# YuHang-max/3DSAD-main

Hardware: AMD Instinct MI355X
Metric: scenes/sec (16384-pt KITTI-shaped) through SA+cluster path (higher is better)
Workload: dtype f32

## Files before the change

### 3dsad-main_amd/_lib.py

```python
import ctypes
import os
import subprocess

_HERE = os.path.dirname(os.path.abspath(__file__))
CSRC = os.path.join(_HERE, "csrc")
SO_PATH = os.environ.get("SAD_AMD_LIB") or os.path.join(CSRC, "libsad_amd.so")

MAX_LAYERS = 4
MAX_RADII = 4
ABI_VERSION = 4
WS_REFILLS, WS_INUSE, WS_CONFLICT = 5, 6, 7

c_f32p = ctypes.POINTER(ctypes.c_float)
c_i32p = ctypes.POINTER(ctypes.c_int32)
vp = ctypes.c_void_p
c_i3p = ctypes.POINTER(ctypes.c_int)


class MlpArgs(ctypes.Structure):
    _fields_ = [
        ("struct_size", ctypes.c_size_t),
        ("xyz", vp), ("new_xyz", vp), ("idx", vp), ("cnt", vp), ("workspace", vp), ("feat", vp),
        ("ld_feat", ctypes.c_int),
        ("B", ctypes.c_int), ("N", ctypes.c_int), ("M", ctypes.c_int), ("S", ctypes.c_int),
# ... 57 lines not shown
        ("struct_size", ctypes.c_size_t),
        ("gt_boxes", vp), ("gt_labels", vp),
        ("B", ctypes.c_int), ("G", ctypes.c_int), ("D", ctypes.c_int), ("H", ctypes.c_int), ("W", ctypes.c_int),
        ("ns", ctypes.c_int), ("nr", ctypes.c_int), ("nb", ctypes.c_int), ("use_size_class", ctypes.c_int),
        ("sizes", ctypes.c_float * 48), ("z_center", ctypes.c_float * 16), ("rotations", ctypes.c_float * 8),
        ("pos_thr", ctypes.c_float * 16), ("neg_thr", ctypes.c_float * 16), ("size_class", ctypes.c_int32 * 16),
        ("x0", ctypes.c_float), ("y0", ctypes.c_float), ("sx", ctypes.c_float), ("sy", ctypes.c_float),
        ("dir_offset", ctypes.c_float),
        ("labels", vp), ("match", vp), ("reg_target", vp), ("max_iou", vp), ("dir_target", vp), ("workspace", vp),
    ]


class CenterTargetsArgs(ctypes.Structure):
    _fields_ = [
        ("struct_size", ctypes.c_size_t),
        ("gt_boxes", vp), ("gt_labels", vp),
        ("B", ctypes.c_int), ("G", ctypes.c_int), ("D", ctypes.c_int), ("C", ctypes.c_int), ("H", ctypes.c_int),
        ("W", ctypes.c_int), ("layout", ctypes.c_int), ("min_radius", ctypes.c_int), ("vel", ctypes.c_int),
        ("lo_x", ctypes.c_float), ("lo_y", ctypes.c_float), ("sx", ctypes.c_float), ("sy", ctypes.c_float),
        ("min_overlap", ctypes.c_float),
        ("heatmap", vp), ("ind", vp), ("anno", vp),
    ]


class AnchorHeadLossArgs(ctypes.Structure):
    _fields_ = [
        ("struct_size", ctypes.c_size_t),
        ("cls", vp), ("reg", vp), ("dir", vp), ("labels", vp), ("reg_target", vp), ("dir_target", vp),
        ("B", ctypes.c_int), ("H", ctypes.c_int), ("W", ctypes.c_int), ("A", ctypes.c_int), ("C", ctypes.c_int),
        ("nb", ctypes.c_int), ("layout", ctypes.c_int), ("sin_diff", ctypes.c_int), ("normalize", ctypes.c_int),
        ("alpha", ctypes.c_float), ("beta", ctypes.c_float),
        ("code_weights", ctypes.c_float * 7), ("scale", ctypes.c_float * 3),
        ("loss", vp), ("num_pos", vp), ("grad_cls", vp), ("grad_reg", vp), ("grad_dir", vp), ("per_anchor", vp),
        ("workspace", vp),
    ]


class CenterHeadLossArgs(ctypes.Structure):
    _fields_ = [
        ("struct_size", ctypes.c_size_t),
        ("hm", vp), ("reg", vp), ("height", vp), ("dim", vp), ("rot", vp), ("vel", vp),
        ("heatmap", vp), ("ind", vp), ("anno", vp),
        ("B", ctypes.c_int), ("H", ctypes.c_int), ("W", ctypes.c_int), ("C", ctypes.c_int), ("G", ctypes.c_int),
        ("layout", ctypes.c_int), ("normalize", ctypes.c_int),
        ("code_weights", ctypes.c_float * 10), ("scale", ctypes.c_float * 2),
        ("loss", vp), ("num_pos", vp),
        ("grad_hm", vp), ("grad_reg", vp), ("grad_height", vp), ("grad_dim", vp), ("grad_rot", vp), ("grad_vel", vp),
        ("workspace", vp),
    ]


ROI_CLS_MODES = {"roi_iou": 0, "cls": 1}


class RoiTargetsArgs(ctypes.Structure):
    _fields_ = [
        ("struct_size", ctypes.c_size_t),
        ("rois", vp), ("roi_count", vp), ("roi_labels", vp), ("gt_boxes", vp), ("gt_labels", vp),
        ("B", ctypes.c_int), ("R", ctypes.c_int), ("D", ctypes.c_int), ("G", ctypes.c_int), ("Dg", ctypes.c_int),
        ("S", ctypes.c_int), ("fg_max", ctypes.c_int), ("cls_mode", ctypes.c_int), ("seed", ctypes.c_uint),
        ("fg_thr", ctypes.c_float), ("bg_lo", ctypes.c_float), ("hard_ratio", ctypes.c_float), ("reg_fg_thr", ctypes.c_float),
        ("cls_fg_thr", ctypes.c_float), ("cls_bg_thr", ctypes.c_float),
        ("index", vp), ("match", vp), ("labels", vp), ("iou", vp), ("cls_target", vp), ("reg_valid", vp),
        ("rois_s", vp), ("gt_local", vp), ("reg_target", vp), ("workspace", vp),
    ]


class RoiHeadLossArgs(ctypes.Structure):
    _fields_ = [
        ("struct_size", ctypes.c_size_t),
        ("rcnn_cls", vp), ("rcnn_reg", vp), ("cls_target", vp), ("reg_valid", vp), ("reg_target", vp), ("rois", vp), ("gt_local", vp),
        ("B", ctypes.c_int), ("S", ctypes.c_int), ("D", ctypes.c_int), ("normalize", ctypes.c_int),
        ("beta", ctypes.c_float), ("code_weights", ctypes.c_float * 7), ("scale", ctypes.c_float * 3),
        ("loss", vp), ("num", vp), ("grad_cls", vp), ("grad_reg", vp), ("grad_corner", vp), ("per_roi", vp),
    ]


SIGNATURES = {
    "sad_version": (ctypes.c_int, []),
    "sad_last_error": (ctypes.c_char_p, []),
    "sad_set_option": (ctypes.c_int, [ctypes.c_char_p, ctypes.c_int]),
    "sad_fps_workspace_bytes": (ctypes.c_size_t, [ctypes.c_int, ctypes.c_int]),
    "sad_fps_f32": (ctypes.c_int, [vp, ctypes.c_int, ctypes.c_int, ctypes.c_int, vp, vp, vp]),
    "sad_ffps_workspace_bytes": (ctypes.c_size_t, [ctypes.c_int, ctypes.c_int]),
    "sad_pairdist_f32": (ctypes.c_int, [vp, vp, ctypes.c_int, ctypes.c_int, ctypes.c_int, ctypes.c_int,
                                       ctypes.c_float, vp, vp]),
    "sad_ffps_f32": (ctypes.c_int, [vp, vp] + [ctypes.c_int] * 5 + [ctypes.c_float, vp, vp, vp]),
    "sad_gather_xyz_f32": (ctypes.c_int, [vp, vp, ctypes.c_int, ctypes.c_int, ctypes.c_int, vp, vp]),
    "sad_gather_points": (ctypes.c_int, [vp, vp] + [ctypes.c_int] * 5 + [vp, vp]),
    "sad_group_points": (ctypes.c_int, [vp, vp] + [ctypes.c_int] * 6 + [vp, vp]),
    "sad_group_points_grad_f32": (ctypes.c_int, [vp, vp] + [ctypes.c_int] * 5 + [vp, vp]),
    "sad_group_points_grad_pm_f32": (ctypes.c_int, [vp, vp] + [ctypes.c_int] * 5 + [vp, vp]),
    "sad_max_pool_s_f32": (ctypes.c_int, [vp] + [ctypes.c_int] * 4 + [vp, vp, vp]),
    "sad_max_pool_s_grad_f32": (ctypes.c_int, [vp, vp] + [ctypes.c_int] * 4 + [vp, vp]),
    "sad_ball_query_f32": (ctypes.c_int, [vp, vp, ctypes.c_float, vp] + [ctypes.c_int] * 4 + [vp, vp]),
    "sad_ball_query_multi_f32": (ctypes.c_int, [vp, vp, ctypes.c_int, c_f32p, vp,
                                               ctypes.POINTER(ctypes.c_int), ctypes.POINTER(vp),
                                               ctypes.POINTER(vp),
                                               ctypes.c_int, ctypes.c_int, ctypes.c_int, vp]),
    "sad_ball_query_grid_workspace_bytes": (ctypes.c_size_t, [ctypes.c_int, ctypes.c_int]),
    "sad_ball_query_grid_f32": (ctypes.c_int, [vp, vp, ctypes.c_int, c_f32p, ctypes.POINTER(ctypes.c_int),
                                              ctypes.POINTER(vp), ctypes.POINTER(vp),
                                              ctypes.c_int, ctypes.c_int, ctypes.c_int, vp, vp]),
    "sad_subsample_pad_f32": (ctypes.c_int, [vp, vp, ctypes.c_int, ctypes.c_int, ctypes.c_int, ctypes.c_uint, vp, vp]),
    "sad_copy_rows_u32": (ctypes.c_int, [vp, ctypes.c_longlong, vp, ctypes.c_longlong, ctypes.c_longlong, ctypes.c_longlong, vp]),
    "sad_knn_f32": (ctypes.c_int, [vp, vp] + [ctypes.c_int] * 4 + [vp, vp]),
    "sad_three_nn_f32": (ctypes.c_int, [vp, vp] + [ctypes.c_int] * 3 + [vp, vp, vp, vp]),
    "sad_three_interpolate_f32": (ctypes.c_int, [vp, vp, vp] + [ctypes.c_int] * 5 + [vp, ctypes.c_int, ctypes.c_int, vp]),
    "sad_three_interpolate_grad_f32": (ctypes.c_int, [vp, vp, vp] + [ctypes.c_int] * 5 + [vp, vp]),
    "sad_boxes_iou_f32": (ctypes.c_int, [vp, vp] + [ctypes.c_int] * 6 + [vp, vp]),
    "sad_points_in_boxes_f32": (ctypes.c_int, [vp, vp] + [ctypes.c_int] * 4 + [vp, vp]),
    "sad_roipoint_pool3d_f32": (ctypes.c_int, [vp, vp, vp] + [ctypes.c_int] * 5 + [ctypes.c_float, ctypes.c_int, vp, vp, vp, vp]),
    "sad_voxel_workspace_bytes": (ctypes.c_int, [ctypes.c_int] * 3 + [ctypes.POINTER(ctypes.c_size_t)]),
    "sad_voxel_coords_f32": (ctypes.c_int, [vp, vp] + [ctypes.c_int] * 3 + [c_f32p, c_f32p, vp, vp]),
    "sad_voxel_index_f32": (ctypes.c_int, [vp, vp] + [ctypes.c_int] * 3 + [c_f32p, c_f32p, ctypes.c_int, vp, vp, vp, vp, vp, vp]),
    "sad_voxelize_f32": (ctypes.c_int, [vp, vp] + [ctypes.c_int] * 3 + [c_f32p, c_f32p, ctypes.c_int, ctypes.c_int, vp, vp, vp, vp, vp, vp]),
    "sad_voxel_reduce_f32": (ctypes.c_int, [vp, vp, vp] + [ctypes.c_int] * 5 + [vp, vp, vp, vp, vp]),
    "sad_voxel_reduce_grad_f32": (ctypes.c_int, [vp, vp, vp] + [ctypes.c_int] * 5 + [vp, vp, vp]),
    "sad_voxel_encode_workspace_bytes": (ctypes.c_int, [ctypes.c_int] * 5 + [ctypes.POINTER(ctypes.c_size_t)]),
    "sad_voxel_decorate_f32": (ctypes.c_int, [vp] * 5 + [ctypes.c_int] * 5 + [c_f32p, c_f32p, ctypes.c_int, ctypes.c_int, vp, vp, vp]),
    "sad_voxel_encode_f32": (ctypes.c_int, [vp] * 5 + [ctypes.c_int] * 5 + [c_f32p, c_f32p, vp, vp] + [ctypes.c_int] * 3 + [vp] * 5),
    "sad_spconv_workspace_bytes": (ctypes.c_int, [ctypes.c_int, ctypes.c_int, c_i3p, c_i3p, ctypes.c_int, ctypes.POINTER(ctypes.c_size_t)]),
    "sad_spconv_index_subm": (ctypes.c_int, [vp, vp, ctypes.c_int, ctypes.c_int, c_i3p, c_i3p, vp, vp, vp]),
    "sad_spconv_index_count": (ctypes.c_int, [vp, vp, ctypes.c_int, ctypes.c_int, c_i3p, c_i3p, c_i3p, c_i3p, vp, vp, vp]),
    "sad_spconv_index_fill": (ctypes.c_int, [vp, vp, ctypes.c_int, ctypes.c_int, c_i3p, c_i3p, c_i3p, c_i3p, vp, ctypes.c_int, vp, vp, vp, vp]),
    "sad_spconv_packed_floats": (ctypes.c_size_t, [ctypes.c_int] * 3),
    "sad_spconv_pack_f32": (ctypes.c_int, [vp, vp] + [ctypes.c_int] * 3 + [vp, vp]),
    "sad_spconv_f32": (ctypes.c_int, [vp, vp, vp, vp] + [ctypes.c_int] * 6 + [vp, vp]),
    "sad_sparse_to_dense_workspace_bytes": (ctypes.c_int, [ctypes.c_int, c_i3p, ctypes.POINTER(ctypes.c_size_t)]),
    "sad_sparse_to_dense_f32": (ctypes.c_int, [vp, vp, vp] + [ctypes.c_int] * 3 + [c_i3p, vp, vp, vp]),
    "sad_spconv_index_transpose": (ctypes.c_int, [vp] + [ctypes.c_int] * 3 + [vp, vp, vp]),
    "sad_spconv_grad_weight_workspace_bytes": (ctypes.c_int, [ctypes.c_int] * 4 + [ctypes.POINTER(ctypes.c_size_t)]),
    "sad_spconv_grad_weight_f32": (ctypes.c_int, [vp, vp, vp] + [ctypes.c_int] * 5 + [vp, vp, vp, vp]),
    "sad_spconv_max_pool_f32": (ctypes.c_int, [vp, vp] + [ctypes.c_int] * 4 + [vp, vp, vp]),
    "sad_spconv_max_pool_grad_f32": (ctypes.c_int, [vp, vp, vp] + [ctypes.c_int] * 4 + [vp, vp]),
    "sad_mlp_packed_floats": (ctypes.c_size_t, [ctypes.c_int, ctypes.POINTER(ctypes.c_int), ctypes.c_int]),
    "sad_mlp_pack_f32": (ctypes.c_int, [ctypes.c_int, ctypes.POINTER(ctypes.c_int), ctypes.c_int,
                                       ctypes.POINTER(vp), ctypes.POINTER(vp), vp, vp]),
    "sad_mlp_workspace_bytes": (ctypes.c_size_t, [ctypes.c_int, ctypes.c_int, ctypes.c_int]),
    "sad_mlp_rowscan": (ctypes.c_int, [ctypes.c_int, ctypes.POINTER(vp), ctypes.POINTER(vp), ctypes.POINTER(ctypes.c_int),
                                       ctypes.c_int, ctypes.c_int, ctypes.c_int, ctypes.POINTER(vp), vp]),
    "sad_mlp_rowscan_init": (ctypes.c_int, [ctypes.c_int, ctypes.POINTER(vp), ctypes.POINTER(vp), ctypes.POINTER(ctypes.c_int),
                                            ctypes.c_int, ctypes.c_int, ctypes.c_int, ctypes.POINTER(vp), ctypes.POINTER(vp),
                                            ctypes.POINTER(ctypes.c_int), ctypes.POINTER(ctypes.c_int), ctypes.POINTER(ctypes.c_int), vp]),
    "sad_mlp_rowscan_split": (ctypes.c_int, [ctypes.c_int, ctypes.POINTER(vp), ctypes.POINTER(vp), ctypes.POINTER(ctypes.c_int),
                                             ctypes.c_int, ctypes.c_int, ctypes.c_int, ctypes.POINTER(vp), ctypes.POINTER(vp),
                                             ctypes.POINTER(ctypes.c_int), vp]),
    "sad_mlp_cont_bytes": (ctypes.c_size_t, [ctypes.c_int] * 4),
    "sad_mlp_preferred_geometry": (ctypes.c_int, [ctypes.c_int, ctypes.POINTER(ctypes.c_int)]),
    "sad_mlp_padded_dims": (ctypes.c_int, [ctypes.c_int, ctypes.POINTER(ctypes.c_int), ctypes.POINTER(ctypes.c_int)]),
    "sad_mlp_scratch_bytes": (ctypes.c_size_t, [ctypes.c_int, ctypes.c_int, ctypes.c_int, ctypes.c_int,
                                               ctypes.POINTER(ctypes.c_int)]),
    "sad_mlp_chain_f32": (ctypes.c_int, [ctypes.POINTER(MlpArgs), vp]),
    "sad_mlp_chain_multi_f32": (ctypes.c_int, [ctypes.POINTER(ctypes.POINTER(MlpArgs)), ctypes.c_int, vp]),
    "sad_mlp_packed_bytes_bf16": (ctypes.c_size_t, [ctypes.c_int, ctypes.POINTER(ctypes.c_int), ctypes.c_int]),
    "sad_mlp_pack_bf16": (ctypes.c_int, [ctypes.c_int, ctypes.POINTER(ctypes.c_int), ctypes.c_int,
                                        ctypes.POINTER(vp), ctypes.POINTER(vp), vp, vp]),
    "sad_mlp_preferred_geometry_bf16": (ctypes.c_int, [ctypes.c_int, ctypes.POINTER(ctypes.c_int)]),
    "sad_mlp_chain_bf16": (ctypes.c_int, [ctypes.POINTER(MlpBf16Args), vp]),
    "sad_mlp_chain_multi_bf16": (ctypes.c_int, [ctypes.POINTER(ctypes.POINTER(MlpBf16Args)), ctypes.c_int, vp]),
    "sad_candidates_f32": (ctypes.c_int, [vp, vp, ctypes.c_int, ctypes.c_int, ctypes.c_int,
                                         ctypes.c_float, ctypes.c_float, ctypes.c_float, c_f32p,
                                         vp, vp, vp]),
    "sad_nms_bev_f32": (ctypes.c_int, [vp, ctypes.c_int, ctypes.c_int, ctypes.c_float, ctypes.c_float,
                                      vp, vp, vp, vp]),
    "sad_nms_bev_workspace_bytes": (ctypes.c_size_t, [ctypes.c_int, ctypes.c_int]),
    "sad_nms_bev_ws_f32": (ctypes.c_int, [vp, ctypes.c_int, ctypes.c_int, ctypes.c_float, ctypes.c_float,
                                         vp, vp, vp, vp, vp]),
    "sad_nms_boxes_workspace_bytes": (ctypes.c_size_t, [ctypes.c_int] * 3),
    "sad_nms_boxes_f32": (ctypes.c_int, [vp, ctypes.c_int, vp, vp, ctypes.c_int, ctypes.c_int, ctypes.c_float, ctypes.c_float,
                                        ctypes.c_int, ctypes.c_int, vp, vp, vp, vp, vp]),
    "sad_decode_boxes_f32": (ctypes.c_int, [vp, vp, ctypes.c_int, ctypes.c_int, c_f32p, vp, vp]),
    "sad_anchor_decode_f32": (ctypes.c_int, [ctypes.POINTER(AnchorDecodeArgs), vp]),
    "sad_center_decode_f32": (ctypes.c_int, [ctypes.POINTER(CenterDecodeArgs), vp]),
    "sad_anchor_targets_workspace_bytes": (ctypes.c_size_t, [ctypes.c_int, ctypes.c_int]),
    "sad_anchor_targets_f32": (ctypes.c_int, [ctypes.POINTER(AnchorTargetsArgs), vp]),
    "sad_center_targets_f32": (ctypes.c_int, [ctypes.POINTER(CenterTargetsArgs), vp]),
    "sad_anchor_head_loss_workspace_bytes": (ctypes.c_size_t, [ctypes.c_int] * 4),
    "sad_anchor_head_loss_f32": (ctypes.c_int, [ctypes.POINTER(AnchorHeadLossArgs), vp]),
    "sad_center_head_loss_workspace_bytes": (ctypes.c_size_t, [ctypes.c_int] * 4),
    "sad_center_head_loss_f32": (ctypes.c_int, [ctypes.POINTER(CenterHeadLossArgs), vp]),
    "sad_roi_targets_workspace_bytes": (ctypes.c_size_t, [ctypes.c_int, ctypes.c_int]),
    "sad_roi_targets_f32": (ctypes.c_int, [ctypes.POINTER(RoiTargetsArgs), vp]),
    "sad_roi_decode_f32": (ctypes.c_int, [vp, ctypes.c_int, vp, ctypes.c_int, ctypes.c_int, vp, vp]),
    "sad_roi_head_loss_f32": (ctypes.c_int, [ctypes.POINTER(RoiHeadLossArgs), vp]),
}

_lib = None

import threading
_tls = threading.local()


def recorder():
    return getattr(_tls, "rec", None)


def set_recorder(rec) -> None:
    _tls.rec = rec


def is_launch(name: str) -> bool:
    return (name.startswith("sad_") and not name.endswith(("_bytes", "_floats", "_bytes_bf16"))
            and "preferred_geometry" not in name and name not in ("sad_version", "sad_last_error", "sad_set_option", "sad_mlp_padded_dims"))


def build(force: bool = False) -> str:
    cmd = ["make", "-C", CSRC, "-j4"] + (["-B"] if force else [])
    subprocess.check_call(cmd, stdout=subprocess.DEVNULL)
    return SO_PATH


def lib():
    global _lib
    if _lib is None:
        if not os.path.exists(SO_PATH):
            raise RuntimeError(
                f"{SO_PATH} is missing: build it with `python -c 'import __graft_entry__ as g; "
                "g.build()'` (hipcc, gfx950).  sad_amd has no CPU fallback.")
        import torch
        handle = ctypes.CDLL(SO_PATH)
        for name, (res, args) in SIGNATURES.items():
            fn = getattr(handle, name)
            fn.restype = res
            fn.argtypes = args
        if handle.sad_version() != ABI_VERSION:
            raise RuntimeError(f"{SO_PATH}: ABI version {handle.sad_version()}, this binding needs {ABI_VERSION} "
                               "(stale build: run __graft_entry__.build())")
        _lib = handle
    rec = getattr(_tls, "rec", None)
    return _lib if rec is None else rec.lib


def check(code: int, what: str) -> None:
    if code != 0:
        msg = lib().sad_last_error()
        raise RuntimeError(f"{what} failed ({code}): {msg.decode() if msg else ''}")


def set_option(key: str, value: int) -> None:
    check(lib().sad_set_option(key.encode(), int(value)), "sad_set_option")
```

### 3dsad-main_amd/csrc/api.hip

```cpp
#include <string.h>

#include "common.h"

namespace sad {

static thread_local char g_err[512] = "";
static std::atomic<int> g_opt[OPT_COUNT] = {};

void set_error(const char *fmt, ...) {
    va_list ap;
    va_start(ap, fmt);
    vsnprintf(g_err, sizeof g_err, fmt, ap);
    va_end(ap);
}

int get_option(int which) { return (which >= 0 && which < OPT_COUNT) ? g_opt[which].load(std::memory_order_relaxed) : 0; }

}

SAD_API int sad_version(void) { return SAD_ABI_VERSION; }

SAD_API const char *sad_last_error(void) { return sad::g_err; }

SAD_API int sad_set_option(const char *key, int value) {
    SAD_REQUIRE(key, "sad_set_option: NULL key");
    if (!strcmp(key, "fps_dpp")) { sad::g_opt[sad::OPT_FPS_DPP].store(value, std::memory_order_relaxed); return SAD_OK; }
    if (!strcmp(key, "mlp_rw")) { sad::g_opt[sad::OPT_MLP_RW].store(value, std::memory_order_relaxed); return SAD_OK; }
    if (!strcmp(key, "mlp_budget_kb")) { sad::g_opt[sad::OPT_MLP_BUDGET_KB].store(value, std::memory_order_relaxed); return SAD_OK; }
    if (!strcmp(key, "mlp_force")) { sad::g_opt[sad::OPT_MLP_FORCE].store(value, std::memory_order_relaxed); return SAD_OK; }
    if (!strcmp(key, "mlp_dedup_f")) { sad::g_opt[sad::OPT_MLP_DEDUP_F].store(value, std::memory_order_relaxed); return SAD_OK; }
    if (!strcmp(key, "mlp_nodedup")) { sad::g_opt[sad::OPT_MLP_NODEDUP].store(value, std::memory_order_relaxed); return SAD_OK; }
    if (!strcmp(key, "mlp_static")) { sad::g_opt[sad::OPT_MLP_STATIC].store(value, std::memory_order_relaxed); return SAD_OK; }
    if (!strcmp(key, "mlp_noxcd")) { sad::g_opt[sad::OPT_MLP_NOXCD].store(value, std::memory_order_relaxed); return SAD_OK; }
    if (!strcmp(key, "mlp_dyn_slots")) { sad::g_opt[sad::OPT_MLP_DYN_SLOTS].store(value, std::memory_order_relaxed); return SAD_OK; }
    if (!strcmp(key, "mlp_steal_after")) { sad::g_opt[sad::OPT_MLP_STEAL_AFTER].store(value, std::memory_order_relaxed); return SAD_OK; }
    if (!strcmp(key, "mlp_layer_queue")) { sad::g_opt[sad::OPT_MLP_LAYER_QUEUE].store(value, std::memory_order_relaxed); return SAD_OK; }
    if (!strcmp(key, "mlp_rows_form")) { sad::g_opt[sad::OPT_MLP_ROWS_FORM].store(value, std::memory_order_relaxed); return SAD_OK; }
    if (!strcmp(key, "mlp_check_inuse")) { sad::g_opt[sad::OPT_MLP_CHECK_INUSE].store(value, std::memory_order_relaxed); return SAD_OK; }
    if (!strcmp(key, "group_variant")) { sad::g_opt[sad::OPT_GROUP_VARIANT].store(value, std::memory_order_relaxed); return SAD_OK; }
    if (!strcmp(key, "bq_variant")) { sad::g_opt[sad::OPT_BQ_VARIANT].store(value, std::memory_order_relaxed); return SAD_OK; }
    if (!strcmp(key, "fps_threads")) { sad::g_opt[sad::OPT_FPS_THREADS].store(value, std::memory_order_relaxed); return SAD_OK; }
    if (!strcmp(key, "nn_variant")) { sad::g_opt[sad::OPT_NN_VARIANT].store(value, std::memory_order_relaxed); return SAD_OK; }
    if (!strcmp(key, "spconv_grad_ranges")) { sad::g_opt[sad::OPT_SPCONV_GRAD_RANGES].store(value, std::memory_order_relaxed); return SAD_OK; }
    if (!strcmp(key, "fps_variant")) { sad::g_opt[sad::OPT_FPS_VARIANT].store(value, std::memory_order_relaxed); return SAD_OK; }
    return sad::fail(SAD_EINVAL, "sad_set_option: unknown key '%s'", key);
}
```

### 3dsad-main_amd/csrc/common.h

```cpp
#pragma once
#include <hip/hip_runtime.h>
#include <atomic>
#include <stdarg.h>
#include <stdint.h>
#include <stdio.h>

#include "../../include/sad_amd.h"

#define SAD_API extern "C" __attribute__((visibility("default")))

namespace sad {

void set_error(const char *fmt, ...);
int get_option(int which);
struct ScanJob {
    const int32_t *cnt, *idx;
    int *tab, *blk_sum, *row_src, *row_gid;
    int ngroups, S, N, M, nodedup, R, blk0;
    float *zout;
    int zld, zcols;
    int split;
    int *gstart;
    void *cont0;
    int cont_cols;
};
struct ScanLayout { long long blk_sum, row_src, row_gid, gstart, ints; };
inline ScanLayout scan_layout(long long ng, int S) {
    ScanLayout t;
    t.blk_sum = 4 + (ng + 1);
    t.row_src = t.blk_sum + (ng * S / 32 + 2) + (ng / 1024 + 2);
    t.row_gid = t.row_src + ng * S;
    t.gstart = (t.row_gid + ng * S + 3) & ~3LL;
    t.ints = t.gstart + ng + 1;
    return t;
}
inline void scan_zero_fill(ScanJob &jb, float *out, int ld_out, int col_off, int cols) { jb.zout = out + col_off; jb.zld = ld_out; jb.zcols = cols; }
inline void heaviest_first(const double *weight, int n, int *order) {
    for (int i = 0; i < n; ++i) order[i] = i;
    for (int i = 0; i < n; ++i)
        for (int k = i + 1; k < n; ++k)
            if (weight[order[k]] > weight[order[i]]) { const int t = order[i]; order[i] = order[k]; order[k] = t; }
}
constexpr int CONT_BIT = 1 << 29;
constexpr int GID_MASK = CONT_BIT - 1;
constexpr int SCAN_MAX_CHAINS = SAD_MAX_RADII;
struct ScanMulti { ScanJob j[SCAN_MAX_CHAINS]; int n; };
ScanJob make_scan_job(const int32_t *cnt, int ngroups, int S, int R, int *tab, int nodedup, const int32_t *idx, int N, int M);
int launch_rowscan_multi(const ScanJob *jobs, int n, hipStream_t st);
int launch_rowscan(const int32_t *cnt, int ngroups, int S, int R, int *tab, hipStream_t st, int nodedup = 0,
                   const int32_t *idx = nullptr, int N = 0, int M = 1);
int launch_fps_cellg(const float *xyz, int B, int N, int M, int32_t *idx, void *workspace, hipStream_t st);
int launch_fps_bucket(const float *xyz, int B, int N, int M, int32_t *idx, void *workspace, hipStream_t st);
constexpr int REG_MAX_CHAINS = 3;
struct RegChain {
    const float *xyz, *new_xyz, *feat, *packed;
    float *out;
    const int *rowtab;
    const int *row_src, *row_gid;
    long long off[3];
    long long stream_off;
    int np[3];
    int ld_feat, C, cpr;
    int ld_out, col_off, cout_last, vec_out;
};
struct RegMulti {
    RegChain c[REG_MAX_CHAINS];
    int shape[REG_MAX_CHAINS];
    int n;
    int *counter;
    int nq;
    long long max_tiles;
    int steal_after;
    int check_id;
};
struct LayerJob {
    const float *x;
    const float *xyz, *new_xyz;
    const int *rowtab, *row_src, *row_gid;
    int rows;
    const float *packed;
    long long off;
    int ldx, np, kg, nog;
    int cpr, gather, relu, last;
    float *y;
    int ldy;
    float *out;
    int ld_out, col_off, cout_last;
};
struct LayerMulti {
    LayerJob j[2];
    int n;
    int *queue;
};
int launch_layers(const LayerMulti &lm, long long max_items, hipStream_t st);
int *stream_item_queue(hipStream_t st);
struct RowsJob {
    const float *x;
    int ldx;
    long long rows;
    const float *packed;
    long long off;
    int np, kg, ct, cout;
    int relu;
    float *out;
    int ld_out, col_off, vec_out;
    int nrb, ncb;
};
int launch_rows(const RowsJob &job, hipStream_t st);
int reg_shape_id(int L, const int *kp, const int *np);
int reg_family(int shape);
int launch_reg(const RegMulti &mp, hipStream_t st);
bool coop_shape(int shape);
long long coop_stream_frags(int shape, const int *kp, const int *np);
int launch_coop(const RegMulti &mp, hipStream_t st);
struct BfRegChain {
    const float *xyz, *new_xyz;
    const void *feat;
    int feat_bf16, ld_feat, C;
    const void *stream;
    int stream_frags;
    const float *bias[3];
    int np[3];
    float *out;
    int ld_out, col_off, cout_last;
    const int *rowtab, *row_src, *row_gid;
    int out_bf16, ld_cont;
    void *cont;
};
struct BfRegMulti {
    BfRegChain c[REG_MAX_CHAINS];
    int shape[REG_MAX_CHAINS];
    int n;
    long long max_tiles;
    int static_f4;
};
struct BfRowsJob {
    const void *x;
    int x_bf16, ldx, kin;
    long long rows;
    const void *w;
    const float *bias;
    int ks, ct, cout;
    int relu;
    void *out;
    int out_bf16, ld_out, col_off, vec_out;
    int nrb, ncb;
    int n_pool;
    const int *pool_gstart[SAD_MAX_RADII];
    const void *pool_cont[SAD_MAX_RADII];
    int pool_col0[SAD_MAX_RADII + 1];
    int pool_ld[SAD_MAX_RADII];
};
int launch_bf16_rows(const BfRowsJob &job, hipStream_t st);
int bfreg_shape_id(int L, const int *dims);
int bfreg_family(int shape);
long long bfreg_stream_frags(int shape);
int bfreg_pack(int shape, const int *dims, int first_has_xyz, const float *const *W, void *dst, hipStream_t st);
int launch_bfreg(const BfRegMulti &mp, hipStream_t st);
enum { OPT_FPS_DPP = 0, OPT_MLP_RW = 1, OPT_MLP_BUDGET_KB = 2, OPT_BQ_VARIANT = 3, OPT_FPS_VARIANT = 4, OPT_MLP_FORCE = 5, OPT_MLP_DEDUP_F = 6, OPT_MLP_NODEDUP = 7, OPT_FPS_THREADS = 8, OPT_MLP_STATIC = 9, OPT_GROUP_VARIANT = 10, OPT_MLP_DYN_SLOTS = 11, OPT_MLP_NOXCD = 12, OPT_MLP_STEAL_AFTER = 13, OPT_MLP_CHECK_INUSE = 14, OPT_MLP_LAYER_QUEUE = 15, OPT_MLP_ROWS_FORM = 16, OPT_NN_VARIANT = 17, OPT_SPCONV_GRAD_RANGES = 18, OPT_COUNT };

inline int fail(int code, const char *fmt, ...) {
    char buf[480];
    va_list ap;
    va_start(ap, fmt);
    vsnprintf(buf, sizeof buf, fmt, ap);
    va_end(ap);
    set_error("%s", buf);
    return code;
}

inline int device_cus() {
    static std::atomic<int> cached{0};
    int c = cached.load(std::memory_order_relaxed);
    if (c > 0) return c;
    int dev = 0;
    c = 256;
    if (hipGetDevice(&dev) == hipSuccess) {
        int v = 0;
        if (hipDeviceGetAttribute(&v, hipDeviceAttributeMultiprocessorCount, dev) == hipSuccess && v > 0) c = v;
    }
    (void)hipGetLastError();
    cached.store(c, std::memory_order_relaxed);
    return c;
}

inline void lds_attr_once(std::atomic<uint64_t> &done, const void *fn, int bytes) {
    int dev = 0;
    if (hipGetDevice(&dev) != hipSuccess) { (void)hipGetLastError(); return; }
    const uint64_t bit = 1ull << (dev & 63);
    if (done.load(std::memory_order_acquire) & bit) return;
    if (hipFuncSetAttribute(fn, hipFuncAttributeMaxDynamicSharedMemorySize, bytes) != hipSuccess) (void)hipGetLastError();
    done.fetch_or(bit, std::memory_order_release);
}

__host__ __device__ inline size_t al16(size_t x) { return (x + 15) & ~(size_t)15; }
struct Carve {
    size_t o = 0;
    size_t take(size_t bytes) { const size_t at = o; o += al16(bytes); return at; }
};
inline unsigned blocks_for(unsigned long long n, int threads) { return (unsigned)((n + threads - 1) / threads); }

inline int check_launch(const char *what) {
    hipError_t e = hipGetLastError();
    if (e != hipSuccess) return fail(SAD_ELAUNCH, "%s: %s", what, hipGetErrorString(e));
    return SAD_OK;
}

constexpr int ITEMQ_REFILLS = 3, ITEMQ_INUSE = 4, ITEMQ_CONFLICT = 5;
struct ItemQueue {
    int *q;
    int nq, own;
};
constexpr int ITEMQ_INTS = 2 + 32 * 8;
__device__ __forceinline__ ItemQueue itemq_init(int *q, int nq) {
    unsigned xcc = 0;
    if (nq == 8) asm volatile("s_getreg_b32 %0, hwreg(HW_REG_XCC_ID)" : "=s"(xcc));
    return ItemQueue{q, nq, (int)(xcc & 7u)};
}
__device__ __forceinline__ int *itemq_counter(const ItemQueue &Q, int x) { return Q.nq == 8 ? Q.q + 2 + 32 * x : Q.q; }
__device__ __forceinline__ int itemq_item(const ItemQueue &Q, int x, int pos) { return Q.nq == 8 ? pos * 8 + x : pos; }
__device__ __forceinline__ int itemq_pull(const ItemQueue &Q, int n = 1) { return atomicAdd(itemq_counter(Q, Q.own), n); }
__device__ __forceinline__ int itemq_steal(const ItemQueue &Q, int nitems) {
    if (Q.nq != 8) return nitems;
    int seen[7];
#pragma unroll
    for (int k = 0; k < 7; ++k)
        seen[k] = __hip_atomic_load(itemq_counter(Q, (Q.own + 1 + k) & 7), __ATOMIC_RELAXED, __HIP_MEMORY_SCOPE_AGENT);
#pragma unroll
    for (int k = 0; k < 7; ++k) {
        const int x = (Q.own + 1 + k) & 7;
        if (itemq_item(Q, x, seen[k]) >= nitems) continue;
        const int it = itemq_item(Q, x, atomicAdd(itemq_counter(Q, x), 1));
        if (it < nitems) return it;
    }
    return nitems;
}
__device__ __forceinline__ void itemq_done(const ItemQueue &Q, int workgroups) {
    if (atomicAdd(Q.q + 1, 1) != workgroups - 1) return;
    Q.q[0] = 0;
    Q.q[1] = 0;
    if (Q.nq == 8) {
        for (int x = 0; x < 8; ++x) Q.q[2 + 32 * x] = 0;
        Q.q[ITEMQ_INUSE] = 0;
    }
}
__device__ __forceinline__ void itemq_claim(const ItemQueue &Q, int id) {
    if (Q.nq != 8 || id == 0) return;
    const int old = atomicCAS(Q.q + ITEMQ_INUSE, 0, id);
    if (old != 0 && old != id) atomicExch(Q.q + ITEMQ_CONFLICT, 1);
}

__device__ __forceinline__ float d2f(float px, float py, float pz, float cx, float cy, float cz) {
    float dx = px - cx, dy = py - cy, dz = pz - cz;
    float xx = dx * dx, yy = dy * dy, zz = dz * dz;
    float s = xx + yy;
    return s + zz;
}

}

#define SAD_REQUIRE(cond, ...)                                \
    do {                                                      \
        if (!(cond)) return sad::fail(SAD_EINVAL, __VA_ARGS__); \
    } while (0)

template <class T> int args_ok(const char *fn, const T *a) {
    SAD_REQUIRE(a, "%s: NULL args", fn);
    SAD_REQUIRE(a->struct_size == sizeof(T), "%s: struct_size %zu, this library has %zu", fn, a->struct_size, sizeof(T));
    return SAD_OK;
}
```

### 3dsad-main_amd/csrc/mlp_chain.h

```cpp
#pragma once
#include "common.h"

namespace sad {
namespace chain {

constexpr int MAXL = SAD_MAX_LAYERS;
constexpr int WHOLE_BIT = 1 << 30;

struct MlpParams {
    const float *xyz;
    const float *new_xyz;
    const int32_t *idx;
    const int32_t *cnt;
    const float *feat;
    const float *packed;
    float *out;
    long long total_rows;
    int ld_feat, N, M, S, C;
    int sp_shift;
    int grouped;
    int L;
    int kp[MAXL];
    int np[MAXL];
    int cout_last;
    long long off[MAXL];
    int relu_mask;
    int ld_out, col_off;
    int wn_shift;
    int xcd_nb;
    int flex;
    int kc;
    int bufA_rows, bufB_rows;
    int cpr, cshift;
    int vec_out;
    int bias_total;
    int G;
    int nodedup;
    int s_off_entries;
    int *rowtab;
    const int *row_src, *row_gid;
    long long total_groups;
};

constexpr int MULTI_MAX = 4;
struct MultiParams {
    MlpParams p[MULTI_MAX];
    int first[MULTI_MAX + 1];
    int rw[MULTI_MAX];
    int cw[MULTI_MAX];
    int n;
};

struct ValuParams {
    const float *xyz, *new_xyz, *feat;
    const int32_t *idx, *cnt;
    const float *w[3], *b[3];
    float *out;
    long long total_groups;
    int ld_feat, N, M, S, G, nodedup, ld_out, col_off, vec_out;
};
constexpr int VALU_T = 256;
constexpr int VALU_GMAX = 2048;

struct Geometry {
    int kp[MAXL], np[MAXL];
    long long off[MAXL];
    long long raw_w[MAXL];
    long long raw_b[MAXL];
    long long stream_off;
    long long stream_frags;
    long long total;
};
Geometry geometry(int L, const int *dims, int first_has_xyz);
int check_dims(const char *fn, int L, const int *dims);

int launch_tiled(const MlpParams &p, int W, int RW, int CW, size_t lds, long long nblocks, hipStream_t st);
int launch_tiled_multi(const MultiParams &mp, int W, int rwmax, bool cw2, size_t lds, hipStream_t st);
int launch_valu(const ValuParams &v, int shape, long long nblocks, hipStream_t st);

}
}
```

### 3dsad-main_amd/csrc/mlp_chain.hip

```cpp
#include "common.h"
#include "mlp_chain.h"

namespace {

using namespace sad::chain;

#include "prims.h"

#ifndef SAD_MLP_BDEPTH
#define SAD_MLP_BDEPTH 2
#endif

__device__ __forceinline__ int act_idx(int c, int r, int PS) {
    return (((c >> 3) << 1) + (c & 1)) * PS + r * 4 + ((c & 7) >> 1);
}

template <int CTRL>
__device__ __forceinline__ float dpp_max(float v) {
    const float o = __builtin_bit_cast(float, __builtin_amdgcn_update_dpp(0, __builtin_bit_cast(int, v), CTRL, 0xF, 0xF, false));
    return o > v ? o : v;
}

__device__ __forceinline__ float group_max(float v, int steps) {
    if (steps > 0) v = dpp_max<0xB1>(v);
// ... 110 lines not shown
                a0[u] = lda(af0, t + D + u, n4);
                a1[u] = lda(af1, t + D + u, n4);
                const int tb = t + u + 2;
                b[u % 2] = bp[(tb < n4 ? tb : n4 - 1) * kbs];
                __builtin_amdgcn_sched_barrier(0);
            }
        }
    }
    const int rem = n4 - t;
#pragma unroll
    for (int u = 0; u < D - 1; ++u) {
        if (u < rem) {
            mma4x2(acc0, acc1, a0[u], a1[u], b[u % 2]);
            if (u + 2 < rem) b[u % 2] = bp[(t + u + 2) * kbs];
        }
    }
}
__device__ __forceinline__ int s_off_last_group(const int *s_off, int G, int T) {
    int lo = 0, hi = G;
    while (hi - lo > 1) {
        const int mid = (lo + hi) >> 1;
        if (s_off[mid] <= T - 1) lo = mid; else hi = mid;
    }
    return lo;
}

template <int W, int RW, int CW = 1>
__device__ __forceinline__ void mlp_chain_body(const MlpParams &p, const int block_in) {
    static_assert(CW == 1 || RW == 1, "two output tiles per wave only with one row tile");
    int block = block_in;
    if (p.xcd_nb > 0) {
        const int per = (p.xcd_nb + 7) >> 3;
        block = (block_in & 7) * per + (block_in >> 3);
        if (block >= p.xcd_nb) return;
    }
    extern __shared__ __attribute__((aligned(16))) float smem[];
    const int tid = threadIdx.x;
    const int lane = tid & 63;
    const int j = lane & 31, h = lane >> 5;
    const int wave = __builtin_amdgcn_readfirstlane(tid >> 6);
    const int WN = 1 << p.wn_shift;
    const int WM = W >> p.wn_shift;
    const int wn = wave & (WN - 1);
    const int wm = wave >> p.wn_shift;
    const int R = 32 * RW * WM;
    const int PS = 4 * R + 8;
    float *bufA = smem;
    float *bufB = smem + (size_t)(p.bufA_rows >> 2) * PS;
    float *sbias = bufB + (size_t)(p.bufB_rows >> 2) * PS;
    int *sm_idx = reinterpret_cast<int *>(sbias + p.bias_total);
    int *sm_gid = sm_idx + R;
    int *s_off = sm_gid + R;
    const int koff = p.grouped ? 4 : 0;

    {
        int bo = 0;
        for (int l = 0; l < p.L; ++l) {
            for (int c = tid; c < p.np[l]; c += W * 64) sbias[bo + c] = p.packed[p.off[l] + c];
            bo += p.np[l];
        }
    }
    long long r0 = (long long)block * R;
    long long g0 = 0;
    int T = R, npass = 1, G = p.G;
    const bool dyn = p.grouped && p.rowtab != nullptr;
    int &s_pass = s_off[p.s_off_entries];
    if (p.grouped && !dyn) {
        g0 = (long long)block * p.G;
        long long left = p.total_groups - g0;
        const int ng = (int)(left < p.G ? left : p.G);
        if (p.cnt) {
            for (int gi = tid; gi < p.G; gi += W * 64) {
                int cnt = 0;
                if (gi < ng) {
                    cnt = p.cnt[g0 + gi];
                    cnt = cnt < 1 ? 1 : (cnt > p.S ? p.S : cnt);
                    if (p.nodedup) cnt = p.S;
                }
                s_off[gi + 1] = cnt;
            }
        } else {
            for (int gi = wave; gi < p.G; gi += W) {
                int cnt = 0;
                if (gi < ng) {
                    const int32_t *ip = p.idx + (g0 + gi) * p.S;
                    const int v = lane < p.S ? ip[lane] : 0;
                    const int first = __builtin_amdgcn_readfirstlane(v);
                    const unsigned long long diff = __ballot(lane < p.S && v != first);
                    cnt = diff ? 64 - __builtin_clzll(diff) : 1;
                    if (p.nodedup) cnt = p.S;
                }
                if (lane == 0) s_off[gi + 1] = cnt;
            }
        }
        if (tid == 0) s_off[0] = 0;
        __syncthreads();
        if (wave == 0) {
            int carry = 0;
            for (int base = 0; base < p.G; base += 64) {
                const int gi = base + lane;
                int v = gi < p.G ? s_off[gi + 1] : 0;
                for (int off = 1; off < 64; off <<= 1) {
                    const int u = __shfl_up(v, off, 64);
                    if (lane >= off) v += u;
                }
                if (gi < p.G) s_off[gi + 1] = v + carry;
                carry += __builtin_amdgcn_readlane(v, 63);
            }
        }
        __syncthreads();
        T = s_off[p.G];
        npass = (T + R - 1) / R;
    }
    const int nchunks = (p.kp[0] + p.kc - 1) / p.kc;

    int next_pass = 0;
    if (dyn && tid == 0) s_pass = atomicAdd(p.rowtab + 2, 1);
    for (int pass_i = 0; dyn || pass_i < npass; ++pass_i) {
        int pass = pass_i;
        int qoff = pass * R;
        if (dyn) {
            __syncthreads();
            pass = s_pass;
            const int total = p.rowtab[0];
            if (pass >= p.rowtab[1]) break;
            T = total - pass * R < R ? total - pass * R : R;
            qoff = 0;
            g0 = 0;
            for (int r = tid; r < R; r += W * 64) {
                const bool valid = r < T;
                const int q = pass * R + (valid ? r : T - 1);
                sm_idx[r] = p.row_src[q];
                const int gv = p.row_gid[q];
                sm_gid[r] = valid ? gv : ~gv;
            }
        }
        for (int r = tid; r < R && !dyn; r += W * 64) {
            if (p.grouped) {
                int q = qoff + r;
                const bool valid = dyn ? r < T : q < T;
                if (!valid) q = T - 1;
                int lo = 0, hi = G;
                while (hi - lo > 1) {
                    const int mid = (lo + hi) >> 1;
                    if (s_off[mid] <= q) lo = mid; else hi = mid;
                }
                const long long gg = g0 + lo;
                const int b = (int)(gg / p.M);
                sm_idx[r] = (int)((long long)b * p.N + p.idx[gg * p.S + (q - s_off[lo])]);
                sm_gid[r] = valid ? lo : -1;
            } else {
                long long gr = r0 + r;
                if (gr >= p.total_rows) gr = p.total_rows - 1;
                sm_idx[r] = (int)gr;
            }
        }
        __syncthreads();
        if (dyn && tid == 0) next_pass = atomicAdd(p.rowtab + 2, 1);

        int bias_off = 0;
        for (int l = 0; l < p.L; ++l) {
            const float *in = (l & 1) ? bufB : bufA;
            float *outb = (l & 1) ? bufA : bufB;
            const int n_oc = p.np[l] >> 5;
            const int nrounds = p.flex ? (n_oc * WM + W * CW - 1) / (W * CW) : (n_oc + WN * CW - 1) / (WN * CW);
            const float4 *frags = reinterpret_cast<const float4 *>(p.packed + p.off[l] + p.np[l]);
            const int nT4 = p.kp[l] >> 3;
            const bool last = (l == p.L - 1);
            const bool relu = (p.relu_mask >> l) & 1;
            const int lchunks = (l == 0) ? nchunks : 1;
            const int keep = last ? p.cout_last : p.kp[l + 1];

            for (int round = 0; round < nrounds; ++round) {
                int ocs[CW];
                bool haves[CW];
                int rtb = wm * RW;
#pragma unroll
                for (int c = 0; c < CW; ++c) {
                    const int item = wave + (round * CW + c) * W;
                    ocs[c] = p.flex ? item / WM : wn + ((round * CW + c) << p.wn_shift);
                    if (p.flex) rtb = item - ocs[c] * WM;
                    haves[c] = ocs[c] < n_oc;
                }
                const bool have = haves[0];
                f32x16 accs[CW][RW];
#pragma unroll
                for (int c = 0; c < CW; ++c) {
                    if (!haves[c]) continue;
#pragma unroll
                    for (int a = 0; a < 4; ++a) {
                        const float4 bv = *reinterpret_cast<const float4 *>(sbias + bias_off + ocs[c] * 32 + 8 * a + 4 * h);
#pragma unroll
                        for (int rt = 0; rt < RW; ++rt) {
                            accs[c][rt][4 * a + 0] = bv.x;
                            accs[c][rt][4 * a + 1] = bv.y;
                            accs[c][rt][4 * a + 2] = bv.z;
                            accs[c][rt][4 * a + 3] = bv.w;
                        }
                    }
                }
                for (int ck = 0; ck < lchunks; ++ck) {
                    const int k0 = (l == 0) ? ck * p.kc : 0;
                    int k1 = (l == 0) ? k0 + p.kc : p.kp[l];
                    if (k1 > p.kp[l]) k1 = p.kp[l];
                    if (l == 0 && (round == 0 || lchunks > 1)) {
                        if (!(round == 0 && ck == 0)) __syncthreads();
                        if (p.grouped && k0 == 0) {
                            for (int r = tid; r < R; r += W * 64) {
                                const int gv = sm_gid[r];
                                const int gi = dyn ? ((gv < 0 ? ~gv : gv) & (WHOLE_BIT - 1))
                                                   : (gv < 0 ? s_off_last_group(s_off, G, T) : gv);
                                const float *q = p.xyz + (long long)sm_idx[r] * 3;
                                const float *c = p.new_xyz + (g0 + gi) * 3;
                                *reinterpret_cast<float2 *>(bufA + r * 4) = make_float2(q[0] - c[0], q[2] - c[2]);
                                *reinterpret_cast<float2 *>(bufA + PS + r * 4) = make_float2(q[1] - c[1], 0.f);
                            }
                        }
                        const int f0 = (k0 > koff ? k0 : koff) - koff;
                        const int f1 = k1 - koff;
                        const int fl = f1 < p.C ? f1 : p.C;
                        if (p.cpr > 0) {
                            const int cprp = 1 << p.cshift;
                            const int rpp = 64 >> p.cshift;
                            for (int r = wave * rpp + (lane >> p.cshift); r < R; r += W * rpp) {
                                const float *src = p.feat + (long long)sm_idx[r] * p.ld_feat;
                                for (int ch = (f0 >> 2) + (lane & (cprp - 1)); ch < (fl >> 2); ch += cprp) {
                                    const float4 v = *reinterpret_cast<const float4 *>(src + 4 * ch);
                                    const int c = koff + 4 * ch - k0;
                                    float *d = bufA + (size_t)((c >> 3) << 1) * PS + r * 4 + ((c & 7) >> 1);
                                    *reinterpret_cast<float2 *>(d) = make_float2(v.x, v.z);
                                    *reinterpret_cast<float2 *>(d + PS) = make_float2(v.y, v.w);
                                }
                            }
                        } else {
                            for (int r = tid; r < R; r += W * 64) {
                                const float *src = p.feat + (long long)sm_idx[r] * p.ld_feat;
                                for (int c = f0; c < fl; ++c) bufA[act_idx(koff + c - k0, r, PS)] = src[c];
                            }
                        }
                        const int z0 = (koff + p.C > k0 ? koff + p.C : k0);
                        for (int k = z0 + wave; k < k1; k += W)
                            for (int r = lane; r < R; r += 64) bufA[act_idx(k - k0, r, PS)] = 0.f;
                        __syncthreads();
                    }
                    if (have) {
                        const float4 *bp = reinterpret_cast<const float4 *>(in) + (size_t)h * (PS >> 2) + rtb * 32 + j;
                        const float4 *af = frags + ((size_t)ocs[0] * nT4 + (k0 >> 3)) * 64 + lane;
                        if constexpr (CW == 2) {
                            if (haves[CW - 1]) {
                                const float4 *af1 = frags + ((size_t)ocs[CW - 1] * nT4 + (k0 >> 3)) * 64 + lane;
                                mma_ktile2<SAD_MLP_ADEPTH>(accs[0][0], accs[CW - 1][0], af, af1, (k1 - k0) >> 3, bp, PS >> 1);
                            } else {
                                mma_ktile<RW, SAD_MLP_ADEPTH>(accs[0], af, (k1 - k0) >> 3, bp, PS >> 1);
                            }
                        } else {
                            mma_ktile<RW, SAD_MLP_ADEPTH>(accs[0], af, (k1 - k0) >> 3, bp, PS >> 1);
                        }
                    }
                }
#pragma unroll
                for (int cw = 0; cw < CW; ++cw) {
                if (!haves[cw]) continue;
                const int oc = ocs[cw];
                f32x16 (&acc)[RW] = accs[cw];
                if (relu) {
#pragma unroll
                    for (int rt = 0; rt < RW; ++rt)
#pragma unroll
                        for (int g = 0; g < 16; ++g) acc[rt][g] = acc[rt][g] > 0.f ? acc[rt][g] : 0.f;
                }
                if (!last) {
#pragma unroll
                    for (int a = 0; a < 4; ++a) {
                        if (oc * 32 + 8 * a >= keep) continue;
#pragma unroll
                        for (int rt = 0; rt < RW; ++rt) {
                            float *d = outb + (size_t)((oc * 4 + a) * 2) * PS + ((rtb + rt) * 32 + j) * 4 + 2 * h;
                            *reinterpret_cast<float2 *>(d) = make_float2(acc[rt][4 * a + 0], acc[rt][4 * a + 2]);
                            *reinterpret_cast<float2 *>(d + PS) = make_float2(acc[rt][4 * a + 1], acc[rt][4 * a + 3]);
                        }
                    }
                } else if (!p.grouped) {
#pragma unroll
                    for (int rt = 0; rt < RW; ++rt) {
                        const long long gr = r0 + (rtb + rt) * 32 + j;
                        if (gr >= p.total_rows) continue;
                        float *o = p.out + gr * p.ld_out + p.col_off;
#pragma unroll
                        for (int a = 0; a < 4; ++a) {
                            const int ch = oc * 32 + 8 * a + 4 * h;
                            if (p.vec_out && ch + 3 < p.cout_last) {
                                *reinterpret_cast<float4 *>(o + ch) = make_float4(acc[rt][4 * a], acc[rt][4 * a + 1], acc[rt][4 * a + 2], acc[rt][4 * a + 3]);
                            } else {
#pragma unroll
                                for (int e = 0; e < 4; ++e)
                                    if (ch + e < p.cout_last) o[ch + e] = acc[rt][4 * a + e];
                            }
                        }
                    }
                } else {
#pragma unroll
                    for (int rt = 0; rt < RW; ++rt) {
                        const int rbase = (rtb + rt) * 32;
                        const int gid = sm_gid[rbase + j];
                        int same[5];
#pragma unroll
                        for (int st = 0; st < 5; ++st) {
// ... 268 lines not shown
```

### 3dsad-main_amd/csrc/mlp_dispatch.hip

```cpp
#include "mlp_chain.h"

using namespace sad::chain;

namespace {
enum Kind { VALU_DONE, TILED, REG, COOP, ROWS, LAYERED };
struct Prepared {
    Kind kind;
    MlpParams p;
    size_t lds;
    long long nblocks;
    int W, RW, CW;
    sad::RegChain rc;
    int reg_shape;
    long long reg_tiles;
    sad::ScanJob scan;
    bool prescanned;
    sad::RowsJob rj;
    sad::LayerJob lj[MAXL];
    int nl;
    long long layer_items[MAXL];
};
struct Chain {
    const sad_mlp_args *a;
    Geometry g;
// ... 228 lines not shown
        return ((size_t)((ra + rb) / 4) * (4 * R + 8) + 2 * R + nso + (size_t)bias_total) * 4 + 16;
    };
    const int bkb = sad::get_option(sad::OPT_MLP_BUDGET_KB);
    const size_t BUDGET2 = (size_t)(bkb > 0 ? bkb : 78) * 1024, BUDGET1 = 156 * 1024;
    int W = 8, wn_shift = 0, RW = 1, kc = g.kp[0];
    if (const int geom = c.geom_wg) {
        const int fw = geom / 100, fwns = (geom / 10) % 10, frw = geom % 10;
        const bool ok = (fw == 4 || fw == 8 || fw == 16) && (1 << fwns) <= fw && (frw == 1 || frw == 2 || frw == 4);
        if (!ok) return sad::fail(SAD_EUNSUPPORTED, "sad_mlp_chain_f32: geometry %d is not valid here", geom);
        W = fw; wn_shift = fwns; RW = frw;
        if (lds_bytes(W, wn_shift, RW, kc) > BUDGET1) {
            kc = g.kp[0] < 256 ? g.kp[0] : 256;
            if (kc == g.kp[0] || lds_bytes(W, wn_shift, RW, kc) > BUDGET1)
                return sad::fail(SAD_EUNSUPPORTED, "sad_mlp_chain_f32: geometry %d does not fit LDS", geom);
        }
    } else {
        double wsum = 0, fsum = 0;
        for (int l = 0; l < a->L; ++l) {
            const double f = (double)g.kp[l] * g.np[l];
            wsum += f * (g.np[l] / 32);
            fsum += f;
        }
        int wns0 = 0;
        while (wns0 < 3 && (2 << wns0) <= wsum / fsum + 1e-9) ++wns0;
        bool found = false;
        for (int pass = 0; pass < 3 && !found; ++pass) {
            const size_t budget = pass == 0 ? BUDGET2 : BUDGET1;
            const int kcc = pass < 2 ? g.kp[0] : (g.kp[0] < 256 ? g.kp[0] : 256);
            for (int wns = wns0; wns <= 3 && !found; ++wns) {
                int best_rw = 0;
                for (int rw = 4; rw >= 1; rw >>= 1) {
                    if (lds_bytes(8, wns, rw, kcc) > budget) continue;
                    if (!best_rw) best_rw = rw;
                    const long long R = 32LL * rw * (8 >> wns);
                    const long long nb = grouped ? (p.total_groups * a->S / dedup_f + R - 1) / R : (p.total_rows + R - 1) / R;
                    if (nb >= 1024 || rw == 1) { best_rw = rw; break; }
                }
                if (best_rw) { wn_shift = wns; RW = best_rw; kc = kcc; found = true; }
            }
        }
        if (!found) return sad::fail(SAD_EUNSUPPORTED, "sad_mlp_chain_f32: layer widths do not fit LDS");
    }
    p.wn_shift = wn_shift;
    if (flex_code > 3 || (flex_code && RW != 1))
        return sad::fail(SAD_EUNSUPPORTED, "sad_mlp_chain_f32: flexible distribution / two tiles per wave need RW == 1");
    if ((flex_code & 2) && W == 16) return sad::fail(SAD_EUNSUPPORTED, "sad_mlp_chain_f32: two tiles per wave: 4 or 8 waves");
    p.flex = flex_code & 1;
    p.kc = kc;
    lds_rows(kc, p.bufA_rows, p.bufB_rows);
    const size_t lds = lds_bytes(W, wn_shift, RW, kc);
    const long long R = 32LL * RW * (W >> wn_shift);
    p.G = grouped ? groups_per_wg((int)R) : 0;
    p.s_off_entries = (int)((p.G > R + 1 ? p.G : R + 1) + 1);
    p.nodedup = sad::get_option(sad::OPT_MLP_NODEDUP);
    p.rowtab = nullptr;
    long long grid_dyn = 0;
    long long macs_per_row = 0;
    for (int l = 0; l < a->L; ++l) macs_per_row += (long long)g.kp[l] * g.np[l];
    const bool want_dyn = c.dyn_code == 1 || (c.dyn_code == 0 && p.total_groups <= 16384 && macs_per_row >= 400000);
    if (grouped && a->cnt && a->workspace && want_dyn && !sad::get_option(sad::OPT_MLP_STATIC)) {
        SAD_REQUIRE((uintptr_t)a->workspace % 16 == 0, "sad_mlp_chain_f32: workspace must be 16-byte aligned");
        SAD_REQUIRE(p.total_groups < (1LL << 30), "sad_mlp_chain_f32: too many groups");
        p.rowtab = (int *)a->workspace;
        if (int e = sad::launch_rowscan(a->cnt, (int)p.total_groups, a->S, (int)R, p.rowtab, (hipStream_t)stream, p.nodedup,
                                        a->idx, a->N, a->M)) return e;
        const sad::ScanLayout t = sad::scan_layout(p.total_groups, a->S);
        p.row_src = p.rowtab + t.row_src;
        p.row_gid = p.rowtab + t.row_gid;
        const long long upper = (p.total_groups * a->S + R - 1) / R;
        long long per_cu = lds > 80 * 1024 ? 1 : (lds > 52 * 1024 ? 2 : (lds > 39 * 1024 ? 3 : 4));
        if (sad::get_option(sad::OPT_MLP_DYN_SLOTS) > 0 && sad::get_option(sad::OPT_MLP_DYN_SLOTS) < per_cu)
            per_cu = sad::get_option(sad::OPT_MLP_DYN_SLOTS);
        grid_dyn = upper < 256 * per_cu ? upper : 256 * per_cu;
    }
    const long long nblocks = grid_dyn ? grid_dyn : (grouped ? (p.total_groups + p.G - 1) / p.G : (p.total_rows + R - 1) / R);
    SAD_REQUIRE(nblocks < (1LL << 31), "sad_mlp_chain_f32: too many workgroups");
    if (W == 16 && RW == 4) return sad::fail(SAD_EUNSUPPORTED, "sad_mlp_chain_f32: 16 waves support RW 1 or 2");
    q.kind = TILED;
    q.p = p; q.lds = lds; q.nblocks = nblocks; q.W = W; q.RW = RW; q.CW = (flex_code & 2) ? 2 : 1;
    if (!grid_dyn && !sad::get_option(sad::OPT_MLP_NOXCD)) {
        q.p.xcd_nb = (int)nblocks;
        q.nblocks = ((nblocks + 7) / 8) * 8;
    }
    return SAD_OK;
}

static int prepare_chain(const sad_mlp_args *a, sad_stream_t stream, Prepared &q) {
    Chain c;
    if (int e = chain_args(a, c)) return e;
    q.prescanned = a->prescanned != 0;
    switch (c.geom_wg) {
    case 1: return prepare_valu(c, stream, q);
    case 2: case 4: return prepare_reg(c, q);
    case 3: return prepare_layered(c, q);
    case 5: return prepare_rows(c, q);
    default: return prepare_tiled(c, stream, q);
    }
}

namespace {
int launch_pending_scans(const Prepared *const *qs, int n, hipStream_t st) {
    sad::ScanJob jobs[sad::REG_MAX_CHAINS];
    int m = 0;
    for (int i = 0; i < n; ++i)
        if (!qs[i]->prescanned) jobs[m++] = qs[i]->scan;
    return m ? sad::launch_rowscan_multi(jobs, m, st) : SAD_OK;
}

int launch_reg_chains(const Prepared *const *qs, int n, hipStream_t st) {
    sad::RegMulti mp{};
    mp.n = n;
    mp.max_tiles = 0;
    if (int e = launch_pending_scans(qs, n, st)) return e;
    for (int i = 0; i < n; ++i) {
        mp.c[i] = qs[i]->rc;
        mp.shape[i] = qs[i]->reg_shape;
        mp.max_tiles += qs[i]->reg_tiles;
    }
    mp.counter = const_cast<int *>(mp.c[0].rowtab) + 2;
    mp.nq = qs[0]->scan.ngroups + 1 >= sad::ITEMQ_INTS ? 8 : 1;
    return qs[0]->kind == COOP ? sad::launch_coop(mp, st) : sad::launch_reg(mp, st);
}

int launch_layered_chains(const Prepared *const *qs, int n, hipStream_t st) {
    if (int e = launch_pending_scans(qs, n, st)) return e;
    for (int l = 0; l < qs[0]->nl; ++l) {
        sad::LayerMulti lm{};
        lm.n = n;
        long long items = 0;
        for (int i = 0; i < n; ++i) { lm.j[i] = qs[i]->lj[l]; items += qs[i]->layer_items[l]; }
        if (int e = sad::launch_layers(lm, items, st)) return e;
    }
    return SAD_OK;
}

int launch_prepared(const Prepared &q, hipStream_t st) {
    const Prepared *one = &q;
    switch (q.kind) {
    case VALU_DONE: return SAD_OK;
    case ROWS: return sad::launch_rows(q.rj, st);
    case LAYERED: return launch_layered_chains(&one, 1, st);
    case REG: case COOP: return launch_reg_chains(&one, 1, st);
    default: return launch_tiled(q.p, q.W, q.RW, q.CW, q.lds, q.nblocks, st);
    }
}
}

SAD_API int sad_mlp_chain_f32(const sad_mlp_args *a, sad_stream_t stream) {
    Prepared q;
    if (int e = prepare_chain(a, stream, q)) return e;
    return launch_prepared(q, (hipStream_t)stream);
}

SAD_API int sad_mlp_chain_multi_f32(const sad_mlp_args *const *args, int n, sad_stream_t stream) {
    SAD_REQUIRE(args && n >= 1, "sad_mlp_chain_multi_f32: need at least one chain");
    hipStream_t st = (hipStream_t)stream;
    if (n > MULTI_MAX) {
        for (int i = 0; i < n; i += MULTI_MAX)
            if (int e = sad_mlp_chain_multi_f32(args + i, n - i < MULTI_MAX ? n - i : MULTI_MAX, stream)) return e;
        return SAD_OK;
    }
    Prepared q[MULTI_MAX];
    for (int i = 0; i < n; ++i)
        if (int e = prepare_chain(args[i], stream, q[i])) return e;
    if (n == 2 && q[0].kind == LAYERED && q[1].kind == LAYERED && q[0].nl == q[1].nl) {
        const int last = q[0].nl - 1;
        const bool swap = q[1].layer_items[last] * (long long)q[1].lj[last].kg > q[0].layer_items[last] * (long long)q[0].lj[last].kg;
        const Prepared *ord[2] = {swap ? &q[1] : &q[0], swap ? &q[0] : &q[1]};
        return launch_layered_chains(ord, 2, st);
    }
    double weight[MULTI_MAX];
    int order[MULTI_MAX];
    bool all_reg = n > 1 && n <= sad::REG_MAX_CHAINS && (q[0].kind == REG || q[0].kind == COOP);
    for (int i = 0; i < n; ++i) all_reg = all_reg && q[i].kind == q[0].kind && sad::reg_family(q[i].reg_shape) == sad::reg_family(q[0].reg_shape);
    if (all_reg) {
        for (int i = 0; i < n; ++i) {
            double m = 0;
            for (int l = 0; l < 3; ++l) m += (double)q[i].rc.np[l] * (l == 0 ? 8.0 * 17 : q[i].rc.np[l - 1]);
            weight[i] = m * (double)q[i].reg_tiles;
        }
        sad::heaviest_first(weight, n, order);
        const Prepared *ord[MULTI_MAX];
        for (int i = 0; i < n; ++i) ord[i] = &q[order[i]];
        return launch_reg_chains(ord, n, st);
    }
    bool merge = n > 1;
    for (int i = 0; i < n; ++i) merge = merge && q[i].kind == TILED && q[i].W == q[0].W && q[i].W != 16;
    if (!merge) {
        for (int i = 0; i < n; ++i)
            if (int e = launch_prepared(q[i], st)) return e;
        return SAD_OK;
    }
    for (int i = 0; i < n; ++i) {
        double m = 0;
        for (int l = 0; l < q[i].p.L; ++l) m += (double)q[i].p.kp[l] * q[i].p.np[l];
        weight[i] = m * (double)q[i].p.total_rows;
    }
    sad::heaviest_first(weight, n, order);
    MultiParams mp{};
    mp.n = n;
    size_t lds = 0;
    long long total = 0;
    int rwmax = 1;
    for (int i = 0; i < n; ++i) {
        const Prepared &s = q[order[i]];
        mp.p[i] = s.p;
        mp.rw[i] = s.RW;
        mp.cw[i] = s.CW;
        mp.first[i] = (int)total;
        total += (s.nblocks + 7) / 8 * 8;
        lds = s.lds > lds ? s.lds : lds;
        rwmax = s.RW > rwmax ? s.RW : rwmax;
    }
    SAD_REQUIRE(total < (1LL << 31), "sad_mlp_chain_multi_f32: too many workgroups");
    mp.first[n] = (int)total;
    bool cw2 = false;
    for (int i = 0; i < n; ++i) cw2 = cw2 || mp.cw[i] == 2;
    return launch_tiled_multi(mp, q[0].W, rwmax, cw2, lds, st);
}
```

### 3dsad-main_amd/csrc/mlp_rowscan.hip

```cpp
#include "mlp_chain.h"

namespace {

using sad::chain::WHOLE_BIT;

constexpr int SCAN_T = 256;
constexpr int SCAN_LOG = 8;
constexpr int SCAN_WAVES = SCAN_T / 64;
static_assert(SCAN_T == 1 << SCAN_LOG, "the row search of rowscan_write_kernel is SCAN_LOG halvings");

__device__ __forceinline__ int scan_job_of(const sad::ScanMulti &sm, int block, int &local) {
    int ji = 0;
    while (ji + 1 < sm.n && block >= sm.j[ji + 1].blk0) ++ji;
    local = block - sm.j[ji].blk0;
    return ji;
}

__device__ __forceinline__ int clamp_cnt(const sad::ScanJob &jb, int g) {
    int c = jb.cnt[g];
    c = c < 1 ? 1 : (c > jb.S ? jb.S : c);
    return jb.nodedup ? jb.S : c;
}

__global__ __launch_bounds__(SCAN_T) void rowscan_sums_kernel(const sad::ScanMulti sm) {
    __shared__ int wsum[SCAN_WAVES];
    int lb;
    const sad::ScanJob &jb = sm.j[scan_job_of(sm, blockIdx.x, lb)];
    const int tid = threadIdx.x, lane = tid & 63, wave = tid >> 6;
    const int g = lb * SCAN_T + tid;
    int c = g < jb.ngroups ? clamp_cnt(jb, g) : 0;
    for (int off = 32; off >= 1; off >>= 1) c += __shfl_xor(c, off, 64);
    if (lane == 0) wsum[wave] = c;
    __syncthreads();
    if (tid == 0) {
        int t = 0;
        for (int w = 0; w < SCAN_WAVES; ++w) t += wsum[w];
        jb.blk_sum[lb] = t;
    }
}

__global__ __launch_bounds__(SCAN_T) void rowscan_write_kernel(const sad::ScanMulti sm) {
    __shared__ int wsum[SCAN_WAVES];
    __shared__ int s_base;
    __shared__ int s_start[SCAN_T + 1];
    int lb;
    const sad::ScanJob &jb = sm.j[scan_job_of(sm, blockIdx.x, lb)];
    const int tid = threadIdx.x, lane = tid & 63, wave = tid >> 6;
    int part = 0;
    for (int b = tid; b < lb; b += SCAN_T) part += jb.blk_sum[b];
    for (int off = 32; off >= 1; off >>= 1) part += __shfl_xor(part, off, 64);
    if (lane == 0) wsum[wave] = part;
    __syncthreads();
    if (tid == 0) {
        int t = 0;
        for (int w = 0; w < SCAN_WAVES; ++w) t += wsum[w];
        s_base = t;
    }
    __syncthreads();
    const int base = s_base;
    const int g = lb * SCAN_T + tid;
    const int c = g < jb.ngroups ? clamp_cnt(jb, g) : 0;
    int incl = c;
    for (int off = 1; off < 64; off <<= 1) {
        const int v = __shfl_up(incl, off, 64);
        if (lane >= off) incl += v;
    }
    __syncthreads();
    if (lane == 63) wsum[wave] = incl;
    __syncthreads();
    int run = incl - c;
    for (int w = 0; w < wave; ++w) run += wsum[w];
    s_start[tid] = run;
    if (tid == SCAN_T - 1) s_start[SCAN_T] = run + c;
    __syncthreads();
    const int blk_rows = s_start[SCAN_T];
    if (jb.split) {
        if (g < jb.ngroups) jb.gstart[g] = base + run;
        if (g == jb.ngroups - 1) jb.gstart[jb.ngroups] = base + run + c;
        if (lb == 0)
            for (int i = tid; i < jb.cont_cols / 2; i += SCAN_T) reinterpret_cast<unsigned *>(jb.cont0)[i] = 0u;
    }
    if (g == jb.ngroups - 1) {
        const int total = base + run + c;
        jb.tab[0] = total;
        jb.tab[1] = (total + jb.R - 1) / jb.R;
        jb.tab[2] = 0;
        jb.tab[3] = 0;
        if (jb.ngroups + 1 >= sad::ITEMQ_INTS) {
            for (int x = 0; x < 8; ++x) jb.tab[4 + 32 * x] = 0;
            jb.tab[2 + sad::ITEMQ_REFILLS] = 0;
            jb.tab[2 + sad::ITEMQ_INUSE] = 0;
            jb.tab[2 + sad::ITEMQ_CONFLICT] = 0;
        }
    }
    if (jb.zout) {
        __shared__ int s_nw[SCAN_T];
        __shared__ int s_nnw;
        if (tid == 0) s_nnw = 0;
        __syncthreads();
        if (g < jb.ngroups) {
            const int r0 = base + run;
            if ((r0 >> 5) != ((r0 + c - 1) >> 5)) s_nw[atomicAdd(&s_nnw, 1)] = g;
        }
        __syncthreads();
        const int nnw = s_nnw;
        if (((jb.zld | jb.zcols) & 3) == 0 && (reinterpret_cast<uintptr_t>(jb.zout) & 15) == 0) {
            const int per = jb.zcols >> 2;
            for (int i = tid; i < nnw * per; i += SCAN_T)
                reinterpret_cast<float4 *>(jb.zout + (long long)s_nw[i / per] * jb.zld)[i % per] = make_float4(0.f, 0.f, 0.f, 0.f);
        } else {
            for (int i = tid; i < nnw * jb.zcols; i += SCAN_T) jb.zout[(long long)s_nw[i / jb.zcols] * jb.zld + i % jb.zcols] = 0.f;
        }
    }
    if (!jb.row_src) return;
    constexpr int U = 4;
    for (int q0 = tid; q0 < blk_rows; q0 += U * SCAN_T) {
        int lo[U], src[U], gid[U];
#pragma unroll
        for (int u = 0; u < U; ++u) {
            const int q = q0 + u * SCAN_T < blk_rows ? q0 + u * SCAN_T : blk_rows - 1;
            int l = 0, h = SCAN_T;
#pragma unroll
            for (int it = 0; it < SCAN_LOG; ++it) {
                const int mid = (l + h) >> 1;
                const bool le = s_start[mid] <= q;
                l = le ? mid : l;
                h = le ? h : mid;
            }
            lo[u] = l;
        }
#pragma unroll
        for (int u = 0; u < U; ++u) {
            const int q = q0 + u * SCAN_T < blk_rows ? q0 + u * SCAN_T : blk_rows - 1;
            const int gg = lb * SCAN_T + lo[u];
            const int r0 = base + s_start[lo[u]], cc = s_start[lo[u] + 1] - s_start[lo[u]];
            const int whole = ((r0 >> 5) == ((r0 + cc - 1) >> 5)) ? WHOLE_BIT : 0;
            const int cont = (jb.split && ((base + q) >> 5) != (r0 >> 5)) ? sad::CONT_BIT : 0;
            const long long b = gg / jb.M;
            src[u] = (int)(b * jb.N + jb.idx[(long long)gg * jb.S + (q - s_start[lo[u]])]);
            gid[u] = gg | whole | cont;
        }
#pragma unroll
        for (int u = 0; u < U; ++u) {
            const int q = q0 + u * SCAN_T;
            if (q < blk_rows) {
                jb.row_src[base + q] = src[u];
                jb.row_gid[base + q] = gid[u];
            }
        }
    }
}
}

namespace sad {
ScanJob make_scan_job(const int32_t *cnt, int ngroups, int S, int R, int *tab, int nodedup, const int32_t *idx, int N, int M) {
    ScanJob jb{};
    jb.cnt = cnt; jb.idx = idx; jb.tab = tab; jb.ngroups = ngroups; jb.S = S; jb.N = N; jb.M = M; jb.nodedup = nodedup; jb.R = R;
    const ScanLayout t = scan_layout(ngroups, S);
    jb.blk_sum = tab + t.blk_sum;
    if (idx) {
        jb.row_src = tab + t.row_src;
        jb.row_gid = tab + t.row_gid;
    }
    jb.gstart = tab + t.gstart;
    return jb;
}

int launch_rowscan_multi(const ScanJob *jobs, int n, hipStream_t st) {
    ScanMulti sm{};
    sm.n = n;
    int blocks = 0;
    for (int i = 0; i < n; ++i) {
        sm.j[i] = jobs[i];
        sm.j[i].blk0 = blocks;
        blocks += (jobs[i].ngroups + SCAN_T - 1) / SCAN_T;
    }
    hipLaunchKernelGGL(rowscan_sums_kernel, dim3(blocks), dim3(SCAN_T), 0, st, sm);
    hipLaunchKernelGGL(rowscan_write_kernel, dim3(blocks), dim3(SCAN_T), 0, st, sm);
#ifdef SAD_SCAN_TWICE
    hipLaunchKernelGGL(rowscan_sums_kernel, dim3(blocks), dim3(SCAN_T), 0, st, sm);
    hipLaunchKernelGGL(rowscan_write_kernel, dim3(blocks), dim3(SCAN_T), 0, st, sm);
#endif
    return check_launch("rowscan");
}

int launch_rowscan(const int32_t *cnt, int ngroups, int S, int R, int *tab, hipStream_t st, int nodedup,
                   const int32_t *idx, int N, int M) {
    const ScanJob jb = make_scan_job(cnt, ngroups, S, R, tab, nodedup, idx, N, M);
    return launch_rowscan_multi(&jb, 1, st);
}
}

enum ScanKind { SCAN_PLAIN, SCAN_INIT, SCAN_SPLIT };
struct ScanArgs {
    int n; const int32_t *const *cnt, *const *idx; const int *S; int B, N, M; void *const *workspace;
    float *const *out; const int *ld_out, *col_off;
    void *const *cont;
    const int *cout;
};
static int rowscan_entry(const char *fn, ScanKind kind, const ScanArgs &a, sad_stream_t stream) {
    const bool arrays = a.cnt && a.idx && a.S && a.workspace && (kind != SCAN_INIT || (a.out && a.ld_out && a.col_off && a.cout)) && (kind != SCAN_SPLIT || (a.cont && a.cout));
    SAD_REQUIRE(a.n >= 1 && a.n <= sad::SCAN_MAX_CHAINS && arrays, "%s: need 1..%d chains and non-NULL arrays", fn, sad::SCAN_MAX_CHAINS);
    const long long max_groups = kind == SCAN_SPLIT ? (long long)sad::CONT_BIT : 1LL << 30;
    SAD_REQUIRE(a.B >= 1 && a.N >= 1 && a.M >= 1 && (long long)a.B * a.M < max_groups, "%s: bad B/N/M", fn);
    sad::ScanJob jobs[sad::SCAN_MAX_CHAINS];
    for (int i = 0; i < a.n; ++i) {
        SAD_REQUIRE(a.cnt[i] && a.idx[i] && a.workspace[i] && a.S[i] >= 1 && a.S[i] <= 64, "%s: chain %d: NULL pointer or bad nsample", fn, i);
        SAD_REQUIRE((uintptr_t)a.workspace[i] % 16 == 0, "%s: workspace must be 16-byte aligned", fn);
        SAD_REQUIRE((long long)a.B * a.M * a.S[i] < (1LL << 31), "%s: B*M*S too large", fn);
        if (kind == SCAN_INIT)
            SAD_REQUIRE(a.out[i] && a.cout[i] >= 1 && a.col_off[i] >= 0 && a.ld_out[i] >= a.col_off[i] + a.cout[i],
                        "%s: chain %d: need out != NULL and col_off + cout <= ld_out", fn, i);
        if (kind == SCAN_SPLIT)
            SAD_REQUIRE(a.cont[i] && (uintptr_t)a.cont[i] % 16 == 0 && a.cout[i] >= 8 && a.cout[i] % 8 == 0,
                        "%s: chain %d: need a 16-byte aligned continuation buffer and cout %% 8 == 0", fn, i);
        jobs[i] = sad::make_scan_job(a.cnt[i], a.B * a.M, a.S[i], 32, (int *)a.workspace[i], kind == SCAN_SPLIT ? 0 : sad::get_option(sad::OPT_MLP_NODEDUP), a.idx[i], a.N, a.M);
        if (kind == SCAN_INIT) sad::scan_zero_fill(jobs[i], a.out[i], a.ld_out[i], a.col_off[i], a.cout[i]);
        if (kind == SCAN_SPLIT) { jobs[i].split = 1; jobs[i].cont0 = a.cont[i]; jobs[i].cont_cols = a.cout[i]; }
    }
    return sad::launch_rowscan_multi(jobs, a.n, (hipStream_t)stream);
}

SAD_API int sad_mlp_rowscan(int n, const int32_t *const *cnt, const int32_t *const *idx, const int *S, int B, int N,
                            int M, void *const *workspace, sad_stream_t stream) {
    return rowscan_entry("sad_mlp_rowscan", SCAN_PLAIN, ScanArgs{n, cnt, idx, S, B, N, M, workspace}, stream);
}

SAD_API int sad_mlp_rowscan_init(int n, const int32_t *const *cnt, const int32_t *const *idx, const int *S, int B, int N,
                                 int M, void *const *workspace, float *const *out, const int *ld_out, const int *col_off,
                                 const int *cout, sad_stream_t stream) {
    ScanArgs a{n, cnt, idx, S, B, N, M, workspace};
    a.out = out; a.ld_out = ld_out; a.col_off = col_off; a.cout = cout;
    return rowscan_entry("sad_mlp_rowscan_init", SCAN_INIT, a, stream);
}

SAD_API int sad_mlp_rowscan_split(int n, const int32_t *const *cnt, const int32_t *const *idx, const int *S, int B, int N,
                                  int M, void *const *workspace, void *const *cont, const int *cout, sad_stream_t stream) {
    ScanArgs a{n, cnt, idx, S, B, N, M, workspace};
    a.cont = cont; a.cout = cout;
    return rowscan_entry("sad_mlp_rowscan_split", SCAN_SPLIT, a, stream);
}

SAD_API size_t sad_mlp_cont_bytes(int B, int M, int S, int cout) {
    if (B < 1 || M < 1 || S < 1 || cout < 1) return 0;
    const size_t tiles = ((size_t)B * M * S + 31) / 32;
    return (tiles + 1) * (size_t)cout * 2;
}

SAD_API size_t sad_mlp_workspace_bytes(int B, int M, int S) {
    if (B < 1 || M < 1 || S < 1) return 0;
    return sizeof(int) * (size_t)sad::scan_layout(B * (long long)M, S).ints + 64;
}
```

### 3dsad-main_amd/detector.py

```python
import ctypes
import math
import os
from typing import Optional

import numpy as np
import torch
from torch import nn

from . import _lib as _libmod
from . import ops
from . import plan as _plan
from ._lib import check, lib
from .config import DetectorConfig
from .sa_module import SAModuleMSG


class SADDetector(nn.Module):
    _streams_created = {}

    def __init__(self, cfg: DetectorConfig, weights: dict, device, overlap_fps: bool = True,
                 n_fps_streams: Optional[int] = None, n_main_streams: int = 2, nested_fps_shortcut: bool = True,
                 dtype: str = "f32", query_on_sampling_stream: bool = True, streams=None, n_extra_streams: int = 2):
        super().__init__()
        if dtype not in ("f32", "bf16"):
# ... 183 lines not shown
            out.append(cur)
        return out

    def _cluster_tables(self, B: int) -> bool:
        cfg = self.cfg
        m3, cin = self.stages[-1].stage.npoint, self.stages[-1].out_channels
        fdt = torch.bfloat16 if (self.dtype == "bf16" and self.stages[-1].agg is not None) else torch.float32
        return all(mlp.wants_prescan(B, m3, cfg.n_cand, s_, self.cluster_cat, cin, feat_dtype=fdt)
                   for mlp, s_ in zip(self.cluster_branches, cfg.cluster_nsamples))

    def _cluster_can_split(self, B: int) -> bool:
        return (self.dtype == "bf16" and ops.SPLIT_POOL and not ops.AUTOTUNE and self.agg_head is None and self._cluster_tables(B)
                and all(mlp.preferred_geometry == 2 and mlp.out_channels % 16 == 0 for mlp in self.cluster_branches)
                and self.cluster_agg.takes_pooled(B * self.cfg.n_cand, self.cluster_agg.out_channels))

    def forward(self, points: torch.Tensor, trace: Optional[dict] = None,
                input_ready: bool = False, ready=None) -> torch.Tensor:
        cfg = self.cfg
        if not points.is_cuda:
            raise RuntimeError("points: expected a GPU tensor (sad_amd has no CPU path)")
        if points.dtype != torch.float32 or points.dim() != 3:
            raise TypeError("points: expected a float32 [B,N,3+C] tensor")
        if not points.is_contiguous():
            ops._unrecordable("points: strided copy")
        points = points.contiguous()
        B, N, D = points.shape
        main = torch.cuda.current_stream()
        rec = _libmod.recorder()
        if rec is not None:
            rec.mark_input(points)

        def new_event(stream):
            if rec is not None:
                return rec.event(stream)
            e = torch.cuda.Event()
            e.record(stream)
            return e

        def wait_for(stream, e):
            if e is None:
                return
            if rec is not None:
                rec.wait(stream, e)
            else:
                stream.wait_event(e)

        def wait_ready(stream):
            if ready is None:
                return
            if rec is not None:
                rec.wait_ready(stream, ready)
            else:
                stream.wait_event(ready)

        wait_ready(main)
        if self.overlap_fps:
            side = self._sides[self._calls % len(self._sides)]
            self._calls += 1
            wait_ready(side)
            if not input_ready:
                ops._unrecordable("forward without input_ready")
                side.wait_stream(main)
            evs = []
            with torch.cuda.stream(side):
                xyz, feat = ops.split_points(points)
                prep = self.query_on_sampling_stream and not ops.AUTOTUNE
                split_ok = prep and trace is None and not self.poison_buffers and self.dtype == "bf16"
                n_in = [N] + [m.stage.npoint for m in self.stages[:-1]]
                splits = []
                for si, m in enumerate(self.stages):
                    prev_agg = si > 0 and self.stages[si - 1].agg is not None
                    splits.append(split_ok and m.can_split(B, n_in[si], m.stage.npoint, feat=feat if si == 0 else None,
                                                           feat_dtype=torch.bfloat16 if prev_agg else torch.float32))
                cluster_tables = self._cluster_tables(B)
                splits.append(split_ok and self._cluster_can_split(B))
                shapes = [(B, m.stage.npoint, m.cat_channels) for m in self.stages]
                shapes.append((B, cfg.n_cand, self.cluster_cat))
                if not prep:
                    ops._unrecordable("zero-filled pooling buffers")
                zeros = (ops._empty if prep else torch.zeros)((sum(a * b_ * c_ for (a, b_, c_), sp in zip(shapes, splits) if not sp),),
                                                              dtype=torch.float32, device=points.device)
                if prep and self.poison_buffers:
                    ops._unrecordable("poisoned buffers")
                    zeros.fill_(float("nan"))
                cats, conts, o = [], [], 0
                for si, (shp, sp) in enumerate(zip(shapes, splits)):
                    if sp:
                        if si < len(self.stages):
                            c_, k_ = self.stages[si].split_buffers(B, shp[1], points.device)
                        else:
                            c_ = ops._empty(shp, dtype=torch.bfloat16, device=points.device)
                            k_ = [ops.cont_buffer(B, shp[1], s_, mlp.out_channels, points.device)
                                  for mlp, s_ in zip(self.cluster_branches, cfg.cluster_nsamples)]
                        cats.append(c_)
                        conts.append(k_)
                        continue
                    n_el = shp[0] * shp[1] * shp[2]
                    cats.append(zeros[o:o + n_el].view(shp))
                    conts.append(None)
                    o += n_el
                if prep and not splits[-1]:
                    if not cluster_tables:
                        ops._unrecordable("zero fill of the cluster pooling buffer")
                        cats[-1].zero_()
                ev_xyz = new_event(side)
                cur = xyz
                centroids = []
                queries = []
                for si in range(len(self.stages)):
                    prev = cur
                    cur = self._sample_stage(si, cur)
                    centroids.append(cur)
                    prev_agg = si > 0 and self.stages[si - 1].agg is not None
                    queries.append(self.stages[si].query(prev, cur, prescan=not ops.AUTOTUNE, cat=cats[si] if prep else None,
                                                         feat=feat if si == 0 else None,
                                                         feat_dtype=torch.bfloat16 if (self.dtype == "bf16" and prev_agg) else torch.float32,
                                                         conts=conts[si])
                                   if self.query_on_sampling_stream else None)
                    evs.append(new_event(side))
            points.record_stream(side)
            for t in centroids + [xyz] + ([feat] if feat is not None else []):
                t.record_stream(main)
            for q in queries:
                if q is not None:
                    for part in q:
                        for t in part:
                            if t is not None:
                                t.record_stream(main)
            zeros.record_stream(main)
            for c_, k_ in zip(cats, conts):
                if k_ is not None:
                    c_.record_stream(main)
                    for t in k_:
                        t.record_stream(main)
            wait_for(main, ev_xyz)
        else:
            xyz, feat = ops.split_points(points)
            centroids = self._sample_chain(xyz)
            evs = [None] * len(centroids)
            queries = [None] * len(centroids)
            cats = [None] * (len(centroids) + 1)
            conts = [None] * (len(centroids) + 1)
        cur_xyz, cur_feat = xyz, feat
        for si, m in enumerate(self.stages):
            wait_for(main, evs[si])
            new_xyz = centroids[si]
            cur_feat = m.group_and_pool(cur_xyz, cur_feat, new_xyz, query=queries[si], cat=cats[si], conts=conts[si],
                                        keep=None if trace is None else trace.setdefault(f"sa{si + 1}", {}))
            if trace is not None:
                trace[f"sa{si + 1}"].update(new_xyz=new_xyz, out=cur_feat)
            cur_xyz = new_xyz
        K = cfg.n_cand
        M3 = cur_xyz.shape[1]
        c = self.cand_mlp.rows(cur_feat if K == M3 else ops.prefix_rows(cur_feat, K))
        cand = ops._empty((B, K, 3), dtype=torch.float32, device=points.device)
        rad = ops._empty((B, K), dtype=torch.float32, device=points.device)
        check(lib().sad_candidates_f32(cur_xyz.data_ptr(), c.data_ptr(), B, M3, K, cfg.shift_max,
                                       cfg.r_min, cfg.r_max, self._anchor, cand.data_ptr(),
                                       rad.data_ptr(), main.cuda_stream), "sad_candidates_f32")
        idxs, cnts = ops.ball_query_multi(cfg.cluster_scales, cfg.cluster_nsamples, cur_xyz, cand, rad,
                                          return_counts=True)
        cat = cats[-1]
        ckont = conts[-1]
        if cat is None and trace is None and not ops.AUTOTUNE and self._cluster_can_split(B):
            cat = ops._empty((B, K, self.cluster_cat), dtype=torch.bfloat16, device=points.device)
            ckont = [ops.cont_buffer(B, K, s_, mlp.out_channels, points.device) for mlp, s_ in zip(self.cluster_branches, cfg.cluster_nsamples)]
        if cat is None:
            ops._unrecordable("zero-filled cluster pooling buffer")
            cat = torch.zeros((B, K, self.cluster_cat), dtype=torch.float32, device=points.device)
        calls, off = [], 0
        cwss = [None] * len(idxs)
        if ckont is not None:
            outs, o_ = [], 0
            for mlp, k_ in zip(self.cluster_branches, ckont):
                outs.append((cat, o_, mlp.out_channels, k_))
                o_ += mlp.out_channels
            cwss = ops.rowscan_multi(idxs, cnts, M3, outs)
        for mlp, idx, cnt, ws, k_ in zip(self.cluster_branches, idxs, cnts, cwss, ckont or [None] * len(idxs)):
            calls.append(ops.GroupedCall(mlp, cur_xyz, cur_feat, cand, idx, out=cat, col_off=off, cnt=cnt, ws=ws, cont=k_))
            off += mlp.out_channels
        ops.grouped_multi(calls)
        if ckont is not None:
            pool = [(w_, k_, s_, mlp.out_channels) for w_, k_, s_, mlp in zip(cwss, ckont, cfg.cluster_nsamples, self.cluster_branches)]
            cfeat = self.cluster_agg.rows(cat, out_dtype=torch.bfloat16, pool=pool)
            o = self.head.rows(cfeat)
        elif self.agg_head is not None and trace is None:
            cfeat = None
            o = self.agg_head.rows(cat)
        else:
            cfeat = (self.cluster_agg.rows(cat, out_dtype=torch.bfloat16) if (self.dtype == "bf16" and trace is None)
                     else self.cluster_agg.rows(cat))
            o = self.head.rows(cfeat)
        boxes = ops._empty((B, K, 9), dtype=torch.float32, device=points.device)
        check(lib().sad_decode_boxes_f32(cand.data_ptr(), o.data_ptr(), B, K, self._anchors,
                                         boxes.data_ptr(), main.cuda_stream), "sad_decode_boxes_f32")
        if trace is not None:
            trace["cluster"] = dict(c=c, cand=cand, radius=rad, ball_idx=idxs, cat=cat, cfeat=cfeat,
                                    head=o)
        return boxes
```

### 3dsad-main_amd/mlp.py

```python
import ctypes
import os
import sys
from typing import Callable, List, NamedTuple, Optional, Sequence, Tuple

import torch

from . import _lib
from ._lib import MlpArgs, check, lib, vp


def rowscan_multi(idxs: Sequence[torch.Tensor], cnts: Sequence[torch.Tensor], N: int,
                  outs: Optional[Sequence[Tuple[torch.Tensor, int, int]]] = None) -> List[torch.Tensor]:
    n = len(idxs)
    if n != len(cnts) or not 1 <= n <= _lib.MAX_RADII:
        raise ValueError(f"need 1..{_lib.MAX_RADII} (idx, cnt) pairs")
    B, M = cnts[0].shape
    wss = []
    for idx, cnt in zip(idxs, cnts):
        idx = ops._need(idx, "idx", torch.int32, 3)
        cnt = ops._need(cnt, "cnt", torch.int32, 2)
        if tuple(idx.shape[:2]) != (B, M) or tuple(cnt.shape) != (B, M):
            raise ValueError("idx / cnt shapes do not match")
        wss.append(ops._empty((lib().sad_mlp_workspace_bytes(B, M, idx.shape[2]),), dtype=torch.uint8, device=idx.device))
    c_arr = (vp * n)(*[c.data_ptr() for c in cnts])
# ... 212 lines not shown
        a.out, a.ld_out, a.col_off = out.data_ptr(), out.stride(-2), col_off


class PackedMLP(_PackedChain):
    _ARGS, _CHAIN = MlpArgs, "sad_mlp_chain_f32"
    _PACK, _PACK_DTYPE = ("sad_mlp_packed_floats", "sad_mlp_pack_f32"), torch.float32

    def __init__(self, layers, first_has_xyz: bool, device, relu_mask: Optional[int] = None,
                 name: str = ""):
        self.preferred_geometry = 0
        ws, bs = self._upload(layers, first_has_xyz, device, relu_mask, name)
        if self.first_has_xyz and self.L == 3 and self.relu_mask == (1 << self.L) - 1:
            pad_c = (ctypes.c_int * (self.L + 1))()
            if lib().sad_mlp_padded_dims(self.L, (ctypes.c_int * (self.L + 1))(*self.dims), pad_c):
                self.pack_dims = [int(v) for v in pad_c]
                for l in range(self.L):
                    w2 = torch.zeros((self.pack_dims[l + 1], self.pack_dims[l]), dtype=torch.float32, device=self.device)
                    w2[:ws[l].shape[0], :ws[l].shape[1]] = ws[l]
                    b2 = torch.zeros((self.pack_dims[l + 1],), dtype=torch.float32, device=self.device)
                    b2[:bs[l].shape[0]] = bs[l]
                    ws[l], bs[l] = w2.contiguous(), b2
        self.padded = self.pack_dims != self.dims
        dims_c = self._pack(ws, bs)
        if self.first_has_xyz:
            self.preferred_geometry = int(lib().sad_mlp_preferred_geometry(self.L, dims_c))
        wide = all(((d + 31) // 32 * 32) % 128 == 0 for d in self.dims[1:])
        self._layered_ok = (not self.padded) and wide and (self.first_has_xyz or (self.dims[0] % 8 == 0 and self.dims[-1] % 128 == 0))

    _CANDIDATES = [w * 100 + n * 10 + r for w in (8, 4) for n in range(4) if (1 << n) <= w
                   for r in (1, 2, 4)] + [1600 + n * 10 + r for n in (3, 4) for r in (1, 2)] \
        + [100000 + w * 100 + n * 10 + 1 for w in (8, 4) for n in range(3) if (2 << n) <= w] \
        + [200000 + w * 100 + n * 10 + 1 for w in (8, 4) for n in range(4) if (1 << n) <= w] \
        + [300000 + w * 100 + n * 10 + 1 for w in (8, 4) for n in range(3) if (2 << n) <= w]
    _F_CODES = (2, 4, 5, 6)

    @staticmethod
    def _takes_table(geom: int) -> bool:
        return geom % 1000 in (2, 3, 4)

    def _launch(self, a: MlpArgs, keep=None) -> None:
        key = self._key(a)
        geom = self._geom.get(key)
        if geom is None and ops.AUTOTUNE:
            geom = self._tune(a)
            self._geom[key] = geom
        a.geometry = geom or self.default_geometry or a.geometry
        _dispatch(self.name, self._CHAIN, self._enqueue(a), keep, retry=lambda: self._drop_untuned_pick(a, geom))

    def _drop_untuned_pick(self, a: MlpArgs, tuned) -> bool:
        if tuned or self.default_geometry or a.geometry <= 5:
            return False
        self.preferred_geometry = 0
        a.geometry = 0
        return True

    def _tune(self, a: MlpArgs) -> int:
        stream = torch.cuda.current_stream()
        enqueue = self._enqueue(a)

        def time(code: int) -> Optional[float]:
            a.geometry = code
            return _time_launch(enqueue, stream)
        best, best_ms = 0, None
        plain_extra = ([3] if self._layered_ok else []) + ([5] if self.L == 1 and self.dims[0] % 8 == 0 else [])
        for code in self._CANDIDATES + ([1] if a.idx else plain_extra):
            ms = time(code)
            if ms is not None and (best_ms is None or ms < best_ms * 0.98):
                best, best_ms = code, ms
        if a.idx and a.cnt and a.workspace:
            t_best, t_ms = 0, None
            for code in (2, 3, 4):
                ms = time(code)
                if ms is not None and (t_ms is None or ms < t_ms * 0.98):
                    t_best, t_ms = code, ms
            if os.environ.get("SAD_TUNE_DEBUG"):
                print(f"[tune] {self.name}: tiled {best} {best_ms}, table {t_best} {t_ms}", file=sys.stderr, flush=True)
            if t_ms is not None and (best_ms is None or t_ms <= best_ms * 1.10):
                return t_best
        if a.idx and best > 4:
            base = best
            for f in self._F_CODES:
                ms = time(base + 1000 * f)
                if ms is not None and ms < best_ms * 0.98:
                    best, best_ms = base + 1000 * f, ms
            if a.cnt and a.workspace:
                base, found = best, None
                for d in (1, 2):
                    ms = time(base + 10000 * d)
                    if ms is not None and (found is None or ms < found[1]):
                        found = (base + 10000 * d, ms)
                if found is not None:
                    best = found[0]
        return best

    def _args(self) -> MlpArgs:
        a = super()._args()
        a.c_out = self.dims[-1] if self.padded else 0
        return a

    @staticmethod
    def feat_fits_table_kernels(C: int, ld_feat: int, ptr: int) -> bool:
        return C <= 1 or (C % 4 == 0 and ld_feat % 4 == 0 and ptr % 16 == 0)

    def _feat_fits(self, feat_pm) -> bool:
        return feat_pm is None or self.feat_fits_table_kernels(feat_pm.shape[2], feat_pm.stride(1), feat_pm.data_ptr())

    def _fresh_fits(self, C: int, dtype) -> bool:
        return self.feat_fits_table_kernels(C, C, 0)

    def grouped(self, xyz: torch.Tensor, feat_pm: Optional[torch.Tensor], new_xyz: torch.Tensor,
                idx: torch.Tensor, out: Optional[torch.Tensor] = None, col_off: int = 0,
                cnt: Optional[torch.Tensor] = None, ws: Optional[torch.Tensor] = None) -> torch.Tensor:
        a, out, _keep = self._grouped_args(xyz, feat_pm, new_xyz, idx, out, col_off, cnt, ws)
        self._launch(a, _keep + [out])
        return out

    @staticmethod
    def _feat_arg(a, feat_pm) -> None:
        if not feat_pm.is_cuda or feat_pm.dtype != torch.float32 or feat_pm.dim() != 3:
            raise TypeError("feat_pm: expected a GPU float32 [B,N,C] tensor")

    def _grouped_args(self, xyz, feat_pm, new_xyz, idx, out, col_off, cnt, ws=None):
        a, keep, xyz, feat_pm = self._grouped_prologue(xyz, feat_pm, new_xyz, idx)
        feat_ok16 = self._feat_fits(feat_pm)
        if self.padded:
            if cnt is None:
                ops._unrecordable("padded chain: counts derived from idx")
                pos = torch.arange(1, a.S + 1, device=idx.device, dtype=torch.int32)
                cnt = torch.clamp(((idx != idx[..., :1]).to(torch.int32) * pos).amax(-1), min=1).to(torch.int32).contiguous()
            if not feat_ok16:
                ops._unrecordable("padded chain: packed copy of the features")
                feat_pm = feat_pm.contiguous()
                a.feat, a.ld_feat = feat_pm.data_ptr(), feat_pm.stride(1)
                keep.append(feat_pm)
                feat_ok16 = self._feat_fits(feat_pm)
        out = self._zero_out(a, xyz.device) if out is None else out
        if self.relu_mask != (1 << self.L) - 1:
            raise RuntimeError("grouped chains need a ReLU after every layer (max-pool combine)")
        self._check_out(out, a.B * a.M, col_off)
        if cnt is not None:
            self._counts_and_table(a, keep, cnt, ws, xyz.device)
        a.out, a.ld_out, a.col_off = out.data_ptr(), out.stride(-2), col_off
        self._pick_geometry(a, cnt is not None and feat_ok16)
        if self._layered_ok and cnt is not None and (a.geometry == 3 or ops.AUTOTUNE):
            self._scratch(a, keep, xyz.device)
        return a, out, keep

    def _scratch(self, a: MlpArgs, keep: list, device) -> None:
        nbytes = lib().sad_mlp_scratch_bytes(a.B, a.M, a.S, self.L, (ctypes.c_int * (self.L + 1))(*self.dims))
        sc = ops._empty((nbytes,), dtype=torch.uint8, device=device)
        a.scratch, a.scratch_bytes = sc.data_ptr(), nbytes
        keep.append(sc)

    def rows(self, x: torch.Tensor, out: Optional[torch.Tensor] = None, col_off: int = 0
             ) -> torch.Tensor:
        if self.first_has_xyz:
            raise RuntimeError("this PackedMLP was packed with the xyz prefix")
        if not x.is_cuda or x.dtype != torch.float32:
            raise TypeError("x: expected a GPU float32 tensor")
        ops._on_current_device(x, "x")
        x2, R, C = self._rows_input(x)
        if out is None:
            out = ops._empty(tuple(x.shape[:-1]) + (self.out_channels,), dtype=torch.float32,
                             device=x.device)
        self._check_out(out, R, col_off)
        a = self._args()
        self._rows_args(a, x2, out, col_off)
        geom = self._geom.get(self._key(a)) or self.default_geometry
        keep = [x2, out]
        if self._layered_ok and self.L > 1 and (geom == 3 or ops.AUTOTUNE):
            self._scratch(a, keep, x.device)
        self._launch(a, keep)
        return out

    def _check_out(self, out: torch.Tensor, rows: int, col_off: int) -> None:
        if not out.is_cuda or out.dtype != torch.float32 or out.stride(-1) != 1:
            raise TypeError("out: expected a GPU float32 tensor with unit last-dim stride")
        if out.numel() // out.shape[-1] != rows or not out.is_contiguous():
            raise ValueError("out: expected a contiguous [rows, ld_out] buffer")
        if col_off < 0 or col_off + self.out_channels > out.shape[-1]:
            raise ValueError("out: col_off + C_out exceeds the buffer width")


class GroupedCall(NamedTuple):
    mlp: _PackedChain
    xyz: torch.Tensor
    feat_pm: Optional[torch.Tensor]
    new_xyz: torch.Tensor
    idx: torch.Tensor
    out: torch.Tensor
    col_off: int
    cnt: Optional[torch.Tensor]
    ws: Optional[torch.Tensor] = None
    cont: Optional[torch.Tensor] = None

    def args(self, table: bool = True):
        more = {} if self.cont is None or not table else {"cont": self.cont}
        return self.mlp._grouped_args(self.xyz, self.feat_pm, self.new_xyz, self.idx, self.out, self.col_off, self.cnt,
                                      self.ws if table else None, **more)


def _multi(calls, args):
    bf16 = isinstance(calls[0].mlp, PackedMLPBf16)
    fn_name = "sad_mlp_chain_multi_bf16" if bf16 else "sad_mlp_chain_multi_f32"
    arr = (ctypes.POINTER(_lib.MlpBf16Args if bf16 else MlpArgs) * len(args))(*[ctypes.pointer(a) for a in args])
    return fn_name, lambda: getattr(lib(), fn_name)(arr, len(args), ops._stream())


def grouped_multi(calls) -> None:
    calls = [GroupedCall(*c) for c in calls]
    if ops.AUTOTUNE or len(calls) < 2 or (not ops.MERGE_BF16 and isinstance(calls[0].mlp, PackedMLPBf16)):
        for c in calls:
            more = {} if c.cont is None else {"ws": c.ws, "cont": c.cont}
            c.mlp.grouped(c.xyz, c.feat_pm, c.new_xyz, c.idx, out=c.out, col_off=c.col_off, cnt=c.cnt, **more)
        if ops.AUTOTUNE and len(calls) >= 2:
            _tune_stage(calls)
        return
    args, keep = [], []
    for c in calls:
        a, _, k = c.args()
        args.append(a)
        keep.append(k)
    bf16 = isinstance(calls[0].mlp, PackedMLPBf16)
    if any(isinstance(c.mlp, PackedMLPBf16) != bf16 for c in calls):
        raise TypeError("grouped_multi: all chains must be of the same class (f32 or bf16)")
    _rec = _lib.recorder()
    if _rec is not None:
        _rec.keep.append((args, keep))
    fn_name, enqueue = _multi(calls, args)
    _dispatch("+".join(c.mlp.name for c in calls), fn_name, enqueue, (keep, [c.out for c in calls]),
              retry=None if bf16 else lambda: any([c.mlp._drop_untuned_pick(a, c.mlp._geom) for a, c in zip(args, calls)]))


def choose_stage_assignment(picked, t_picked, uniform_times, table=(2, 3, 4)):
    u_best, u_t = None, None
    for code in table:
        t = uniform_times.get(code)
        if t is not None and (u_t is None or t < u_t * 0.98):
            u_best, u_t = code, t
    all_table = all(p in table for p in picked)
    if u_t is not None:
        if (all_table and (t_picked is None or u_t < t_picked * 0.98)) or (not all_table and (t_picked is None or u_t <= t_picked * 1.10)):
            return [u_best] * len(picked), u_t
    return list(picked), t_picked


def _tune_stage(calls) -> None:
    calls = [GroupedCall(*c) for c in calls]
    stream = torch.cuda.current_stream()
    bf16 = isinstance(calls[0].mlp, PackedMLPBf16)
    keys = [c.mlp._key(c.args(table=False)[0]) for c in calls]

    def run(codes):
        args, keep = [], []
        for c, code in zip(calls, codes):
            a, _, k = c.args(table=False)
            a.geometry = code
            args.append(a)
            keep.append(k)
        return _time_launch(_multi(calls, args)[1], stream)

    picked = [c.mlp._geom.get(k) or 0 for c, k in zip(calls, keys)]
    table = (2,) if bf16 else (2, 3, 4)
    all_table = all(p in table for p in picked)
    t_picked = run(picked)
    uniform = {}
    for code in table:
        uniform[code] = t_picked if (all_table and all(p == code for p in picked)) else run([code] * len(calls))
    best, t_best = choose_stage_assignment(picked, t_picked, uniform, table)
    if os.environ.get("SAD_TUNE_DEBUG"):
        print(f"[tune-stage] {'+'.join(c.mlp.name for c in calls)}: picked {picked} {t_picked}, uniform {uniform}, final {best} {t_best}", file=sys.stderr, flush=True)
    for c, k, code in zip(calls, keys, best):
        c.mlp._geom[k] = code


class PackedMLPBf16(_PackedChain):
    _ARGS, _CHAIN = _lib.MlpBf16Args, "sad_mlp_chain_bf16"
    _PACK, _PACK_DTYPE = ("sad_mlp_packed_bytes_bf16", "sad_mlp_pack_bf16"), torch.uint8

    def __init__(self, layers, first_has_xyz: bool, device, relu_mask: Optional[int] = None,
                 name: str = ""):
        dims_c = self._pack(*self._upload(layers, first_has_xyz, device, relu_mask, name))
        self.preferred_geometry = int(lib().sad_mlp_preferred_geometry_bf16(self.L, dims_c)) if self.first_has_xyz else 0

    @staticmethod
    def _takes_table(geom: int) -> bool:
        return geom == 2

    def _feat_ok_reg(self, feat_pm) -> bool:
        if feat_pm is None:
            return True
        C = feat_pm.shape[2]
        if C <= 13:
            return True
        return (feat_pm.dtype == torch.bfloat16 and C % 8 == 0 and feat_pm.stride(1) % 8 == 0 and feat_pm.data_ptr() % 16 == 0)

    _feat_fits = _feat_ok_reg

    def _fresh_fits(self, C: int, dtype) -> bool:
        return C <= 13 or (dtype in (None, torch.bfloat16) and C % 8 == 0)

    @staticmethod
    def _feat(t: torch.Tensor, name: str):
        if not t.is_cuda or t.dtype not in (torch.bfloat16, torch.float32):
            raise TypeError(f"{name}: expected a GPU bfloat16 or float32 tensor")
        return 1 if t.dtype == torch.bfloat16 else 0

    def grouped(self, xyz: torch.Tensor, feat_pm: Optional[torch.Tensor], new_xyz: torch.Tensor,
                idx: torch.Tensor, out: Optional[torch.Tensor] = None, col_off: int = 0,
                cnt: Optional[torch.Tensor] = None, ws: Optional[torch.Tensor] = None,
                cont: Optional[torch.Tensor] = None) -> torch.Tensor:
        a, out, _keep = self._grouped_args(xyz, feat_pm, new_xyz, idx, out, col_off, cnt, ws, cont)
        self._launch(a, _keep + [out])
# ... 101 lines not shown
```

### 3dsad-main_amd/ops.py

```python
import ctypes
import os
from typing import Optional, Sequence, Tuple, Union

import numpy as np
import torch

from . import _lib
from ._lib import check, lib, vp


def _stream() -> int:
    return torch.cuda.current_stream().cuda_stream


def _empty(*a, **k) -> torch.Tensor:
    rec = _lib.recorder()
    return torch.empty(*a, **k) if rec is None else rec.empty(*a, **k)


def _unrecordable(what: str) -> None:
    if _lib.recorder() is not None:
        from .plan import PlanUnsupported
        raise PlanUnsupported(what)


def copy_rows(src: torch.Tensor, src_off_words: int, src_stride_words: int, n_rows: int, row_words: int,
              out: torch.Tensor, dst_stride_words: Optional[int] = None) -> torch.Tensor:
    check(lib().sad_copy_rows_u32(src.data_ptr() + 4 * int(src_off_words), int(src_stride_words), out.data_ptr(),
                                  int(row_words if dst_stride_words is None else dst_stride_words), int(n_rows), int(row_words),
                                  _stream()), "sad_copy_rows_u32")
    return out


def copy_to_host(src: torch.Tensor, dst_pinned: torch.Tensor) -> None:
    if not src.is_cuda or not src.is_contiguous() or dst_pinned.is_cuda or not dst_pinned.is_pinned() or not dst_pinned.is_contiguous():
        raise TypeError("copy_to_host: expected a contiguous GPU source and a contiguous pinned host destination")
    nbytes = src.numel() * src.element_size()
    if nbytes != dst_pinned.numel() * dst_pinned.element_size() or nbytes % 4 != 0:
        raise ValueError("copy_to_host: sizes differ (or are not whole 4-byte words)")
    check(lib().sad_copy_rows_u32(src.data_ptr(), nbytes // 4, dst_pinned.data_ptr(), nbytes // 4, 1, nbytes // 4, _stream()),
          "sad_copy_rows_u32")


def split_points(points: torch.Tensor):
    B, N, D = points.shape
    xyz = _empty((B, N, 3), dtype=torch.float32, device=points.device)
    copy_rows(points, 0, D, B * N, 3, xyz)
    feat = None
    if D > 3:
        feat = _empty((B, N, D - 3), dtype=torch.float32, device=points.device)
        copy_rows(points, 3, D, B * N, D - 3, feat)
    return xyz, feat


def prefix_rows(x: torch.Tensor, m: int) -> torch.Tensor:
    B, M, C = x.shape
    rb = C * x.element_size()
    if rb % 4 != 0 or not x.is_contiguous() or not x.is_cuda:
        raise TypeError("prefix_rows: expected a contiguous GPU tensor whose rows are whole 4-byte words")
    out = _empty((B, m, C), dtype=x.dtype, device=x.device)
    return copy_rows(x, 0, M * rb // 4, B, m * rb // 4, out)


LAUNCH_LOG: Optional[list] = None
RERUN_LOG: Optional[list] = None

GRID_MIN_POINTS: int = 2048

AUTOTUNE: bool = False
MERGE_BF16: bool = True
SPLIT_POOL: bool = not os.environ.get("SAD_NO_SPLIT_POOL")


class _timed:
    __slots__ = ("kind", "name", "ev")

    def __init__(self, kind: str, name: str = ""):
        self.kind, self.name, self.ev = kind, name, None

    def __enter__(self):
        if LAUNCH_LOG is not None:
            self.ev = torch.cuda.Event(enable_timing=True)
            self.ev.record(torch.cuda.current_stream())
        return self

    def __exit__(self, *exc):
        if self.ev is not None:
            end = torch.cuda.Event(enable_timing=True)
            end.record(torch.cuda.current_stream())
            LAUNCH_LOG.append((self.kind, self.name, self.ev, end))
        return False


def _on_current_device(t: torch.Tensor, name: str) -> None:
    cur = torch.cuda.current_device()
    if t.device.index != cur:
        raise RuntimeError(f"{name}: tensor is on {t.device} but the current device is cuda:{cur}; "
                           f"wrap the call in `with torch.cuda.device({t.device.index}):`")


def _need(t: torch.Tensor, name: str, dtype, ndim: int) -> torch.Tensor:
    if not isinstance(t, torch.Tensor):
        raise TypeError(f"{name}: expected a torch.Tensor")
    if not t.is_cuda:
        raise RuntimeError(f"{name}: expected a GPU tensor (sad_amd has no CPU path)")
    _on_current_device(t, name)
    if dtype is not None and t.dtype != dtype:
        raise TypeError(f"{name}: expected dtype {dtype}, got {t.dtype}")
    if t.dim() != ndim:
        raise ValueError(f"{name}: expected {ndim} dims, got shape {tuple(t.shape)}")
    if not t.is_contiguous():
        _unrecordable(f"{name}: strided copy")
    return t.contiguous()


def _f32(v) -> float:
    return float(np.float32(v))


def _ptr(t: Optional[torch.Tensor]):
    return t.data_ptr() if t is not None else None


def _results(*ts):
    res = tuple(t for t in ts if t is not None)
    return res[0] if len(res) == 1 else res


def _offsets(offsets: torch.Tensor, dev, of: str) -> int:
    if offsets.device != dev:
        raise ValueError(f"offsets must be on the device of {of}")
    B = offsets.shape[0] - 1
    if B < 1:
        raise ValueError("offsets must have B + 1 >= 2 entries")
    return B


def _outputs(spec, out: Optional[tuple], dev, of: str) -> tuple:
    if out is None:
        return tuple(_empty(shape, dtype=dt, device=dev) for _, shape, dt in spec)
    ok = len(out) == len(spec) and all(isinstance(t, torch.Tensor) and tuple(t.shape) == tuple(shape) and t.dtype == dt
                                       and t.is_contiguous() and t.device == dev for t, (_, shape, dt) in zip(out, spec))
    if not ok:
        want = ", ".join(f"{n} {list(shape)} {str(dt).replace('torch.', '')}" for n, shape, dt in spec)
        raise ValueError(f"out: expected contiguous ({want}) on the device of {of}")
    return tuple(out)


def _bytes(fn_name: str, *args) -> int:
    n = ctypes.c_size_t(0)
    check(getattr(lib(), fn_name)(*args, ctypes.byref(n)), fn_name)
    return n.value


def _workspace(nbytes: int, given: Optional[torch.Tensor], dev, maker: str, align: int = 1) -> torch.Tensor:
    if given is None:
        return _empty((nbytes,), dtype=torch.uint8, device=dev)
    if (not isinstance(given, torch.Tensor) or not given.is_cuda or given.device != dev or not given.is_contiguous()
            or given.numel() * given.element_size() < nbytes or given.data_ptr() % align):
        raise ValueError(f"workspace: expected a contiguous GPU buffer of at least {nbytes} bytes on {dev}"
                         + (f", {align}-byte aligned" if align > 1 else "") + f" ({maker})")
    return given


def fps(xyz: torch.Tensor, npoint: int) -> torch.Tensor:
    xyz = _need(xyz, "xyz", torch.float32, 3)
    B, N, three = xyz.shape
    if three != 3:
        raise ValueError("xyz: last dim must be 3")
    if not 1 <= npoint <= N:
        raise ValueError(f"npoint={npoint} must be in 1..N={N}")
    idx = _empty((B, npoint), dtype=torch.int32, device=xyz.device)
    ws_bytes = lib().sad_fps_workspace_bytes(B, N)
    ws = _empty((ws_bytes,), dtype=torch.uint8, device=xyz.device) if ws_bytes else None
    with _timed("fps", f"N{N}"):
        check(lib().sad_fps_f32(xyz.data_ptr(), B, N, npoint, idx.data_ptr(), _ptr(ws), _stream()), "sad_fps_f32")
    return idx


def ffps(xyz: torch.Tensor, feat_pm: torch.Tensor, npoint: int, w_xyz: float = 1.0) -> torch.Tensor:
    xyz = _need(xyz, "xyz", torch.float32, 3)
    feat_pm = _need(feat_pm, "feat_pm", torch.float32, 3)
    B, N, _ = xyz.shape
    if feat_pm.shape[0] != B or feat_pm.shape[1] != N:
        raise ValueError("feat_pm must be [B,N,C]")
    if feat_pm.stride(2) != 1 or feat_pm.stride(0) != N * feat_pm.stride(1):
        feat_pm = feat_pm.contiguous()
    if not 1 <= npoint <= N:
        raise ValueError(f"npoint={npoint} must be in 1..N={N}")
    idx = _empty((B, npoint), dtype=torch.int32, device=xyz.device)
    ws = _empty((lib().sad_ffps_workspace_bytes(B, N),), dtype=torch.uint8, device=xyz.device)
    with _timed("fps", f"F{N}"):
        check(lib().sad_ffps_f32(xyz.data_ptr(), feat_pm.data_ptr(), feat_pm.stride(1), B, N,
                                 feat_pm.shape[2], npoint, float(w_xyz), idx.data_ptr(), ws.data_ptr(),
                                 _stream()), "sad_ffps_f32")
    return idx


def dfps_ffps(xyz: torch.Tensor, feat_pm: torch.Tensor, npoint: int, w_xyz: float = 1.0) -> torch.Tensor:
    half = npoint // 2
    parts = ([fps(xyz, half)] if half else []) + [ffps(xyz, feat_pm, npoint - half, w_xyz)]
    return torch.cat(parts, dim=1)


def gather_xyz(xyz: torch.Tensor, idx: torch.Tensor) -> torch.Tensor:
    xyz = _need(xyz, "xyz", torch.float32, 3)
    idx = _need(idx, "idx", torch.int32, 2)
    B, N, _ = xyz.shape
    M = idx.shape[1]
    out = _empty((B, M, 3), dtype=torch.float32, device=xyz.device)
    check(lib().sad_gather_xyz_f32(xyz.data_ptr(), idx.data_ptr(), B, N, M, out.data_ptr(), _stream()),
          "sad_gather_xyz_f32")
    return out


def gather_points(features: torch.Tensor, idx: torch.Tensor) -> torch.Tensor:
    features = _need(features, "features", None, 3)
    idx = _need(idx, "idx", torch.int32, 2)
    esz = features.element_size()
    if esz not in (2, 4):
        raise TypeError("features: element size must be 2 or 4 bytes")
    B, C, N = features.shape
    M = idx.shape[1]
    out = _empty((B, C, M), dtype=features.dtype, device=features.device)
    check(lib().sad_gather_points(features.data_ptr(), idx.data_ptr(), B, C, N, M, esz,
                                  out.data_ptr(), _stream()), "sad_gather_points")
    return out


def group_points(features: torch.Tensor, idx: torch.Tensor) -> torch.Tensor:
    features = _need(features, "features", None, 3)
    idx = _need(idx, "idx", torch.int32, 3)
    esz = features.element_size()
    if esz not in (2, 4):
        raise TypeError("features: element size must be 2 or 4 bytes")
    B, C, N = features.shape
    _, M, S = idx.shape
    out = _empty((B, C, M, S), dtype=features.dtype, device=features.device)
    with _timed("group_points", f"C{C}N{N}M{M}S{S}"):
        check(lib().sad_group_points(features.data_ptr(), idx.data_ptr(), B, C, N, M, S, esz,
                                     out.data_ptr(), _stream()), "sad_group_points")
    return out


def subsample_pad(points: torch.Tensor, offsets: torch.Tensor, n_points: int, seed: int = 0,
                  out: Optional[torch.Tensor] = None) -> torch.Tensor:
    points = _need(points, "points", torch.float32, 2)
    offsets = _need(offsets, "offsets", torch.int32, 1)
    B = _offsets(offsets, points.device, "points")
    C = points.shape[1]
    out, = _outputs((("out", (B, n_points, C), torch.float32),), None if out is None else (out,), points.device, "points")
    check(lib().sad_subsample_pad_f32(points.data_ptr(), offsets.data_ptr(), B, C, int(n_points),
                                      int(seed) & 0xFFFFFFFF, out.data_ptr(), _stream()), "sad_subsample_pad_f32")
    return out


def ball_query(radius: Union[float, torch.Tensor], nsample: int, xyz: torch.Tensor,
               new_xyz: torch.Tensor) -> torch.Tensor:
    xyz = _need(xyz, "xyz", torch.float32, 3)
    new_xyz = _need(new_xyz, "new_xyz", torch.float32, 3)
    B, N, _ = xyz.shape
    M = new_xyz.shape[1]
    if new_xyz.shape[0] != B:
        raise ValueError("xyz / new_xyz batch mismatch")
    idx = _empty((B, M, nsample), dtype=torch.int32, device=xyz.device)
    if isinstance(radius, torch.Tensor):
        rad = _need(radius, "radius", torch.float32, 2)
        if tuple(rad.shape) != (B, M):
            raise ValueError(f"radius tensor must be [B,M]=({B},{M})")
        check(lib().sad_ball_query_f32(xyz.data_ptr(), new_xyz.data_ptr(), 0.0, rad.data_ptr(), B, N, M,
                                       nsample, idx.data_ptr(), _stream()), "sad_ball_query_f32")
    else:
        check(lib().sad_ball_query_f32(xyz.data_ptr(), new_xyz.data_ptr(), _f32(radius), None, B, N, M, nsample, idx.data_ptr(), _stream()),
              "sad_ball_query_f32")
    return idx


def ball_query_multi(radii: Sequence[float], nsamples: Sequence[int], xyz: torch.Tensor,
                     new_xyz: torch.Tensor, radius_pc: Optional[torch.Tensor] = None,
                     return_counts: bool = False):
    xyz = _need(xyz, "xyz", torch.float32, 3)
    new_xyz = _need(new_xyz, "new_xyz", torch.float32, 3)
    B, N, _ = xyz.shape
    M = new_xyz.shape[1]
    n = len(radii)
    if n != len(nsamples) or not 1 <= n <= _lib.MAX_RADII:
        raise ValueError(f"need 1..{_lib.MAX_RADII} radii with matching nsamples")
    outs = [_empty((B, M, s), dtype=torch.int32, device=xyz.device) for s in nsamples]
    r_arr = (ctypes.c_float * n)(*[_f32(r) for r in radii])
    s_arr = (ctypes.c_int * n)(*[int(s) for s in nsamples])
    p_arr = (vp * n)(*[o.data_ptr() for o in outs])
    cnts = [_empty((B, M), dtype=torch.int32, device=xyz.device) for _ in nsamples] if return_counts else None
    c_arr = (vp * n)(*[c.data_ptr() for c in cnts]) if return_counts else None
    pc = None
    if radius_pc is not None:
        radius_pc = _need(radius_pc, "radius_pc", torch.float32, 2)
        if tuple(radius_pc.shape) != (B, M):
            raise ValueError(f"radius_pc must be [B,M]=({B},{M})")
        pc = radius_pc.data_ptr()
    if pc is None and N >= GRID_MIN_POINTS and N <= 65536 and min(radii) > 0:
        ws = _empty((lib().sad_ball_query_grid_workspace_bytes(B, N),), dtype=torch.uint8,
                         device=xyz.device)
        with _timed("ball_query", f"N{N}M{M}x{n}"):
            check(lib().sad_ball_query_grid_f32(xyz.data_ptr(), new_xyz.data_ptr(), n, r_arr, s_arr, p_arr,
                                                c_arr, B, N, M, ws.data_ptr(), _stream()),
                  "sad_ball_query_grid_f32")
        return (outs, cnts) if return_counts else outs
    with _timed("ball_query", f"N{N}M{M}x{n}"):
        check(lib().sad_ball_query_multi_f32(xyz.data_ptr(), new_xyz.data_ptr(), n, r_arr, pc, s_arr,
                                             p_arr, c_arr, B, N, M, _stream()), "sad_ball_query_multi_f32")
    return (outs, cnts) if return_counts else outs


def knn_query(k: int, xyz: torch.Tensor, new_xyz: torch.Tensor) -> torch.Tensor:
    xyz = _need(xyz, "xyz", torch.float32, 3)
    new_xyz = _need(new_xyz, "new_xyz", torch.float32, 3)
    B, N, _ = xyz.shape
    M = new_xyz.shape[1]
    idx = _empty((B, M, k), dtype=torch.int32, device=xyz.device)
    check(lib().sad_knn_f32(xyz.data_ptr(), new_xyz.data_ptr(), B, N, M, k, idx.data_ptr(), _stream()),
          "sad_knn_f32")
    return idx


def three_nn(unknown: torch.Tensor, known: torch.Tensor) -> Tuple[torch.Tensor, torch.Tensor, torch.Tensor]:
    unknown = _need(unknown, "unknown", torch.float32, 3)
    known = _need(known, "known", torch.float32, 3)
    B, n, three = unknown.shape
    if three != 3 or known.shape[2] != 3 or known.shape[0] != B:
        raise ValueError("unknown [B,n,3] and known [B,m,3] expected")
    m = known.shape[1]
    dist2 = _empty((B, n, 3), dtype=torch.float32, device=unknown.device)
    idx = _empty((B, n, 3), dtype=torch.int32, device=unknown.device)
    w = _empty((B, n, 3), dtype=torch.float32, device=unknown.device)
    with _timed("three_nn", f"n{n}m{m}"):
        check(lib().sad_three_nn_f32(unknown.data_ptr(), known.data_ptr(), B, n, m, dist2.data_ptr(), idx.data_ptr(),
                                     w.data_ptr(), _stream()), "sad_three_nn_f32")
    return dist2, idx, w


def three_interpolate(feat: torch.Tensor, idx: torch.Tensor, w: torch.Tensor, point_major: bool = False,
                      out: Optional[torch.Tensor] = None, col_off: int = 0) -> torch.Tensor:
    feat = _need(feat, "feat", torch.float32, 3)
    idx = _need(idx, "idx", torch.int32, 3)
    w = _need(w, "w", torch.float32, 3)
    B, n = idx.shape[0], idx.shape[1]
    if idx.shape[2] != 3 or tuple(w.shape) != tuple(idx.shape) or feat.shape[0] != B:
        raise ValueError("idx and w must be [B,n,3] and feat must have the same B")
    C, m = (feat.shape[2], feat.shape[1]) if point_major else (feat.shape[1], feat.shape[2])
    if point_major:
        if out is None:
            if col_off != 0:
                raise ValueError("col_off needs an out buffer")
            out = _empty((B, n, C), dtype=torch.float32, device=feat.device)
        if (not out.is_cuda or out.dtype != torch.float32 or not out.is_contiguous() or out.dim() != 3
                or tuple(out.shape[:2]) != (B, n) or out.device != feat.device):
            raise ValueError("out: expected a contiguous float32 [B,n,ld] tensor on the device of feat")
        ld = out.shape[2]
    else:
        if out is not None or col_off != 0:
            raise ValueError("out / col_off apply to the point-major layout only")
        out = _empty((B, C, n), dtype=torch.float32, device=feat.device)
        ld = n
    with _timed("three_interpolate", f"C{C}" + ("pm" if point_major else "cm")):
        check(lib().sad_three_interpolate_f32(feat.data_ptr(), idx.data_ptr(), w.data_ptr(), B, C, m, n, int(bool(point_major)),
                                              out.data_ptr(), ld, int(col_off), _stream()), "sad_three_interpolate_f32")
    return out


def _boxes(t: torch.Tensor, name: str, batched: bool = True) -> torch.Tensor:
    t = _need(t, name, torch.float32, 3 if batched else 2)
    if t.shape[-1] < 7:
        raise ValueError(f"{name}: box rows need at least 7 fields (cx,cy,cz,l,w,h,yaw), got {t.shape[-1]}")
    return t


def _boxes_iou(a: torch.Tensor, b: torch.Tensor, mode: int, kind: str) -> torch.Tensor:
    batched = isinstance(a, torch.Tensor) and a.dim() == 3
    a = _boxes(a, "a", batched)
    b = _boxes(b, "b", batched)
    if not batched:
        a, b = a.unsqueeze(0), b.unsqueeze(0)
    B, Ka, Da = a.shape
    if b.shape[0] != B or b.device != a.device:
        raise ValueError("a and b must have the same batch size and device")
    Kb, Db = b.shape[1], b.shape[2]
    iou = _empty((B, Ka, Kb), dtype=torch.float32, device=a.device)
    with _timed("boxes_iou", f"{kind}Ka{Ka}Kb{Kb}"):
        check(lib().sad_boxes_iou_f32(a.data_ptr(), b.data_ptr(), B, Ka, Kb, Da, Db, mode, iou.data_ptr(), _stream()),
              "sad_boxes_iou_f32")
    return iou if batched else iou[0]


def boxes_iou_bev(a: torch.Tensor, b: torch.Tensor) -> torch.Tensor:
    return _boxes_iou(a, b, 0, "bev")


def boxes_iou3d(a: torch.Tensor, b: torch.Tensor) -> torch.Tensor:
    return _boxes_iou(a, b, 1, "3d")


def _xyz_boxes(xyz: torch.Tensor, boxes: torch.Tensor):
    xyz = _need(xyz, "xyz", torch.float32, 3)
    boxes = _boxes(boxes, "boxes")
    B, N, three = xyz.shape
    if three != 3 or boxes.shape[0] != B or boxes.device != xyz.device:
        raise ValueError("xyz [B,N,3] and boxes [B,K,D] on one device expected")
    return xyz, boxes, B, N, boxes.shape[1], boxes.shape[2]


def points_in_boxes(xyz: torch.Tensor, boxes: torch.Tensor) -> torch.Tensor:
    xyz, boxes, B, N, K, D = _xyz_boxes(xyz, boxes)
    box_idx = _empty((B, N), dtype=torch.int32, device=xyz.device)
    with _timed("points_in_boxes", f"N{N}K{K}"):
        check(lib().sad_points_in_boxes_f32(xyz.data_ptr(), boxes.data_ptr(), B, N, K, D, box_idx.data_ptr(), _stream()),
              "sad_points_in_boxes_f32")
    return box_idx


def roipoint_pool3d(xyz: torch.Tensor, feat_pm: Optional[torch.Tensor], boxes: torch.Tensor, extra_width: float,
                    num_sampled_points: int, return_idx: bool = False):
    xyz, boxes, B, N, K, D = _xyz_boxes(xyz, boxes)
    C = 0
    if feat_pm is not None:
        feat_pm = _need(feat_pm, "feat_pm", torch.float32, 3)
        if tuple(feat_pm.shape[:2]) != (B, N) or feat_pm.device != xyz.device:
            raise ValueError("feat_pm: expected [B,N,C] on the device of xyz")
        C = feat_pm.shape[2]
    S = int(num_sampled_points)
    if S < 1:
        raise ValueError(f"num_sampled_points={S} must be >= 1")
    pooled = _empty((B, K, S, 3 + C), dtype=torch.float32, device=xyz.device)
    empty = _empty((B, K), dtype=torch.int32, device=xyz.device)
    idx = _empty((B, K, S), dtype=torch.int32, device=xyz.device) if return_idx else None
    with _timed("roipoint_pool3d", f"N{N}K{K}S{S}C{C}"):
        check(lib().sad_roipoint_pool3d_f32(xyz.data_ptr(), feat_pm.data_ptr() if C else None, boxes.data_ptr(), B, N, K, D, C,
                                            _f32(extra_width), S, pooled.data_ptr(), empty.data_ptr(), _ptr(idx), _stream()),
              "sad_roipoint_pool3d_f32")
    return (pooled, empty, idx) if return_idx else (pooled, empty)


VOXEL_MODES = {"sum": 0, "mean": 1, "max": 2}


def _voxel_points(points: torch.Tensor, offsets: Optional[torch.Tensor], name: str = "points", min_c: int = 3):
    if offsets is None:
        points = _need(points, name, torch.float32, 3)
        B, N, C = points.shape
        if B < 1:
            raise ValueError(f"{name}: empty batch")
        if B * N >= 1 << 30:
            raise ValueError(f"{name}: too many points")
        offsets = torch.arange(0, (B + 1) * N, N, dtype=torch.int32, device=points.device) if N else \
            torch.zeros((B + 1,), dtype=torch.int32, device=points.device)
        points = points.view(B * N, C)
    else:
        points = _need(points, name, torch.float32, 2)
        offsets = _need(offsets, "offsets", torch.int32, 1)
        B = _offsets(offsets, points.device, name)
    if points.shape[1] < min_c:
        raise ValueError(f"{name}: rows need at least {min_c} columns, got {points.shape[1]}")
    return points, offsets, B


# ... 1029 lines not shown
```

### include/sad_amd.h

```cpp
#ifndef SAD_AMD_H
#define SAD_AMD_H

#include <stddef.h>
#include <stdint.h>

#ifdef __cplusplus
extern "C" {
#endif

#define SAD_OK 0
#define SAD_EINVAL (-1)
#define SAD_EUNSUPPORTED (-2)
#define SAD_ELAUNCH (-3)

#define SAD_MAX_LAYERS 4
#define SAD_MAX_RADII 4

typedef void *sad_stream_t;

#define SAD_ABI_VERSION 4
int sad_version(void);
const char *sad_last_error(void);
#define SAD_WS_REFILLS 5
#define SAD_WS_INUSE 6
// ... 13 lines not shown
int sad_gather_xyz_f32(const float *xyz, const int32_t *idx, int B, int N, int M, float *out,
                       sad_stream_t stream);
int sad_gather_points(const void *src, const int32_t *idx, int B, int C, int N, int M,
                      int elem_size, void *out, sad_stream_t stream);
int sad_group_points(const void *feat, const int32_t *idx, int B, int C, int N, int M, int S,
                     int elem_size, void *out, sad_stream_t stream);

int sad_group_points_grad_f32(const float *grad_out, const int32_t *idx, int B, int C, int N, int M,
                              int S, float *grad_feat, sad_stream_t stream);
int sad_group_points_grad_pm_f32(const float *grad_out, const int32_t *idx, int B, int C, int N,
                                 int M, int S, float *grad_feat_pm, sad_stream_t stream);
int sad_max_pool_s_f32(const float *x, int B, int C, int M, int S, float *out, int32_t *arg,
                       sad_stream_t stream);
int sad_max_pool_s_grad_f32(const float *grad_out, const int32_t *arg, int B, int C, int M, int S,
                            float *grad_x, sad_stream_t stream);

int sad_ball_query_f32(const float *xyz, const float *new_xyz, float radius,
                       const float *radius_pc, int B, int N, int M, int S, int32_t *idx,
                       sad_stream_t stream);
int sad_ball_query_multi_f32(const float *xyz, const float *new_xyz, int n_radii,
                             const float *radii, const float *radius_pc, const int *nsamples,
                             int32_t *const *idx, int32_t *const *cnt, int B, int N, int M,
                             sad_stream_t stream);

size_t sad_ball_query_grid_workspace_bytes(int B, int N);
int sad_ball_query_grid_f32(const float *xyz, const float *new_xyz, int n_radii, const float *radii,
                            const int *nsamples, int32_t *const *idx, int32_t *const *cnt, int B,
                            int N, int M, void *workspace, sad_stream_t stream);

int sad_subsample_pad_f32(const float *points, const int32_t *offsets, int B, int C, int n_points,
                          unsigned seed, float *out, sad_stream_t stream);

int sad_copy_rows_u32(const void *src, long long src_stride_words, void *dst, long long dst_stride_words,
                      long long n_rows, long long row_words, sad_stream_t stream);

int sad_three_nn_f32(const float *unknown, const float *known, int B, int n, int m, float *dist2,
                     int32_t *idx, float *w, sad_stream_t stream);
int sad_three_interpolate_f32(const float *feat, const int32_t *idx, const float *w, int B, int C,
                              int m, int n, int point_major, float *out, int ld_out, int col_off,
                              sad_stream_t stream);
int sad_three_interpolate_grad_f32(const float *grad_out, const int32_t *idx, const float *w, int B,
                                   int C, int n, int m, int point_major, float *grad_feat_pm,
                                   sad_stream_t stream);

#define SAD_IOU_BEV 0
#define SAD_IOU_3D 1
int sad_boxes_iou_f32(const float *a, const float *b, int B, int Ka, int Kb, int Da, int Db, int mode,
                      float *iou, sad_stream_t stream);
int sad_points_in_boxes_f32(const float *xyz, const float *boxes, int B, int N, int K, int D,
                            int32_t *box_idx, sad_stream_t stream);
int sad_roipoint_pool3d_f32(const float *xyz, const float *feat, const float *boxes, int B, int N,
                            int K, int D, int C, float extra_width, int S, float *pooled,
                            int32_t *empty, int32_t *idx, sad_stream_t stream);

#define SAD_VOXEL_SUM 0
#define SAD_VOXEL_MEAN 1
#define SAD_VOXEL_MAX 2
int sad_voxel_workspace_bytes(int total_points, int B, int max_voxels, size_t *bytes);
int sad_voxel_coords_f32(const float *points, const int32_t *offsets, int total_points, int B, int C,
                         const float *voxel_size, const float *point_range, int32_t *coors,
                         sad_stream_t stream);
int sad_voxel_index_f32(const float *points, const int32_t *offsets, int total_points, int B, int C,
                        const float *voxel_size, const float *point_range, int max_voxels,
                        int32_t *point2voxel, int32_t *coors, int32_t *count, int32_t *voxel_num,
                        void *workspace, sad_stream_t stream);
int sad_voxelize_f32(const float *points, const int32_t *offsets, int total_points, int B, int C,
                     const float *voxel_size, const float *point_range, int max_points, int max_voxels,
                     float *voxels, int32_t *coors, int32_t *num_points, int32_t *voxel_num,
                     void *workspace, sad_stream_t stream);
int sad_voxel_reduce_f32(const float *feat, const int32_t *point2voxel, const int32_t *offsets,
                         int total_points, int B, int Cf, int max_voxels, int mode, float *out,
                         int32_t *arg, int32_t *count, void *workspace, sad_stream_t stream);
int sad_voxel_reduce_grad_f32(const float *grad_out, const int32_t *point2voxel, const int32_t *offsets,
                              int total_points, int B, int Cf, int max_voxels, int mode,
                              const int32_t *count_or_arg, float *grad_feat, sad_stream_t stream);

#define SAD_VFE_CLUSTER_CENTER 1
#define SAD_VFE_VOXEL_CENTER 2
#define SAD_VFE_RELU 4
int sad_voxel_encode_workspace_bytes(int total_points, int B, int max_voxels, int Cin, int Cout, size_t *bytes);
int sad_voxel_decorate_f32(const float *points, const int32_t *point2voxel, const int32_t *offsets,
                           const int32_t *coors, const float *vox_feat, int total_points, int B, int C,
                           int max_voxels, int Cv, const float *voxel_size, const float *point_range,
                           int flags, int max_points, float *rows, void *workspace, sad_stream_t stream);
int sad_voxel_encode_f32(const float *points, const int32_t *point2voxel, const int32_t *offsets,
                         const int32_t *coors, const float *vox_feat, int total_points, int B, int C,
                         int max_voxels, int Cv, const float *voxel_size, const float *point_range,
                         const float *weight, const float *bias, int Cout, int flags, int max_points,
                         float *pooled, int32_t *arg, float *pointwise, void *workspace, sad_stream_t stream);

int sad_spconv_workspace_bytes(int Nv, int B, const int *kernel, const int *stride, int subm, size_t *bytes);
int sad_spconv_index_subm(const int32_t *coors, const int32_t *offsets, int Nv, int B, const int *spatial_shape,
                          const int *kernel, int32_t *nbr, void *workspace, sad_stream_t stream);
int sad_spconv_index_count(const int32_t *coors, const int32_t *offsets, int Nv, int B, const int *spatial_shape,
                           const int *kernel, const int *stride, const int *padding, int32_t *out_offsets,
                           void *workspace, sad_stream_t stream);
int sad_spconv_index_fill(const int32_t *coors, const int32_t *offsets, int Nv, int B, const int *spatial_shape,
                          const int *kernel, const int *stride, const int *padding, const int32_t *out_offsets,
                          int capacity, int32_t *out_coors, int32_t *nbr, void *workspace, sad_stream_t stream);
size_t sad_spconv_packed_floats(int Kvol, int Cin, int Cout);
int sad_spconv_pack_f32(const float *W, const float *bias, int Kvol, int Cin, int Cout, float *packed,
                        sad_stream_t stream);
int sad_spconv_f32(const float *feat, const int32_t *nbr, const float *packed, const float *residual, int relu,
                   int Nv, int No, int Kvol, int Cin, int Cout, float *out, sad_stream_t stream);
int sad_sparse_to_dense_workspace_bytes(int B, const int *out_shape, size_t *bytes);
int sad_sparse_to_dense_f32(const float *feat, const int32_t *out_coors, const int32_t *out_offsets, int No, int B,
                            int C, const int *out_shape, float *dense, void *workspace, sad_stream_t stream);
int sad_spconv_index_transpose(const int32_t *nbr, int No, int Nv, int Kvol, int32_t *nbrT, int32_t *collisions,
                               sad_stream_t stream);
int sad_spconv_grad_weight_workspace_bytes(int No, int Kvol, int Cin, int Cout, size_t *bytes);
int sad_spconv_grad_weight_f32(const float *feat, const int32_t *nbr, const float *g, int Nv, int No, int Kvol, int Cin,
                               int Cout, float *grad_W, float *grad_bias, void *workspace, sad_stream_t stream);
int sad_spconv_max_pool_f32(const float *feat, const int32_t *nbr, int Nv, int No, int Kvol, int C, float *out, int32_t *arg,
                            sad_stream_t stream);
int sad_spconv_max_pool_grad_f32(const float *g, const int32_t *arg, const int32_t *nbrT, int Nv, int No, int Kvol, int C,
                                 float *grad_feat, sad_stream_t stream);

int sad_knn_f32(const float *xyz, const float *new_xyz, int B, int N, int M, int K, int32_t *idx,
                sad_stream_t stream);

size_t sad_mlp_packed_floats(int L, const int *dims, int first_has_xyz);
int sad_mlp_pack_f32(int L, const int *dims, int first_has_xyz, const float *const *W,
                     const float *const *bias, float *packed, sad_stream_t stream);

typedef struct sad_mlp_args {
    size_t struct_size;
    const float *xyz;
    const float *new_xyz;
    const int32_t *idx;
    const int32_t *cnt;
    void *workspace;
    const float *feat;
    int ld_feat;
    int B, N, M, S, C;
    int L;
    int dims[SAD_MAX_LAYERS + 1];
    const float *packed;
    int relu_mask;
    float *out;
    int ld_out;
    int col_off;
    int geometry;
    void *scratch;
    size_t scratch_bytes;
    int prescanned;
    int c_out;
} sad_mlp_args;
size_t sad_mlp_workspace_bytes(int B, int M, int S);
int sad_mlp_rowscan(int n, const int32_t *const *cnt, const int32_t *const *idx, const int *S, int B, int N,
                    int M, void *const *workspace, sad_stream_t stream);
int sad_mlp_rowscan_init(int n, const int32_t *const *cnt, const int32_t *const *idx, const int *S, int B, int N,
                         int M, void *const *workspace, float *const *out, const int *ld_out, const int *col_off,
                         const int *cout, sad_stream_t stream);
size_t sad_mlp_scratch_bytes(int B, int M, int S, int L, const int *dims);
int sad_mlp_preferred_geometry(int L, const int *dims);
int sad_mlp_padded_dims(int L, const int *dims, int *padded);
int sad_mlp_chain_f32(const sad_mlp_args *args, sad_stream_t stream);
int sad_mlp_chain_multi_f32(const sad_mlp_args *const *args, int n, sad_stream_t stream);

size_t sad_mlp_packed_bytes_bf16(int L, const int *dims, int first_has_xyz);
int sad_mlp_pack_bf16(int L, const int *dims, int first_has_xyz, const float *const *W,
                      const float *const *bias, void *packed, sad_stream_t stream);
typedef struct sad_mlp_bf16_args {
    size_t struct_size;
    const float *xyz;
    const float *new_xyz;
    const int32_t *idx;
    const void *feat;
    int feat_bf16;
    int ld_feat;
    int B, N, M, S, C;
    int L;
    int dims[SAD_MAX_LAYERS + 1];
    const void *packed;
    int relu_mask;
    void *out;
    int out_bf16;
    int ld_out;
    int col_off;
    const int32_t *cnt;
    void *workspace;
    int geometry;
    int prescanned;
    void *cont;
    int n_pool;
    const void *pool_ws[SAD_MAX_RADII];
    const void *pool_cont[SAD_MAX_RADII];
    int pool_S[SAD_MAX_RADII];
    int pool_cols[SAD_MAX_RADII];
} sad_mlp_bf16_args;
size_t sad_mlp_cont_bytes(int B, int M, int S, int cout);
int sad_mlp_rowscan_split(int n, const int32_t *const *cnt, const int32_t *const *idx, const int *S, int B, int N,
                          int M, void *const *workspace, void *const *cont, const int *cout, sad_stream_t stream);
int sad_mlp_preferred_geometry_bf16(int L, const int *dims);
int sad_mlp_chain_bf16(const sad_mlp_bf16_args *args, sad_stream_t stream);
int sad_mlp_chain_multi_bf16(const sad_mlp_bf16_args *const *args, int n, sad_stream_t stream);

int sad_candidates_f32(const float *xyz3, const float *c, int B, int M3, int K, float shift_max,
                       float r_min, float r_max, const float *anchor, float *cand, float *radius,
                       sad_stream_t stream);
int sad_decode_boxes_f32(const float *cand, const float *o, int B, int K, const float *anchors,
                         float *boxes, sad_stream_t stream);

int sad_nms_bev_f32(const float *boxes, int B, int K, float iou_thr, float score_thr, int32_t *keep,
                    int32_t *order, int32_t *count, sad_stream_t stream);
size_t sad_nms_bev_workspace_bytes(int B, int K);
int sad_nms_bev_ws_f32(const float *boxes, int B, int K, float iou_thr, float score_thr, int32_t *keep,
                       int32_t *order, int32_t *count, void *workspace, sad_stream_t stream);

size_t sad_nms_boxes_workspace_bytes(int B, int K, int pre_max);
int sad_nms_boxes_f32(const float *boxes, int D, const float *scores, const int32_t *labels, int B, int K,
                      float iou_thr, float score_thr, int pre_max, int post_max, int32_t *keep, int32_t *order,
                      int32_t *count, void *workspace, sad_stream_t stream);

#define SAD_LAYOUT_NCHW 0
#define SAD_LAYOUT_NHWC 1

typedef struct sad_anchor_decode_args {
    size_t struct_size;
    const float *cls, *reg, *dir;
    const int32_t *index;
    int B, H, W, C, nb, ns, nr, layout, P;
    float sizes[48];
    float z_center[16];
    float rotations[8];
    float x0, y0, sx, sy;
    float dir_offset, dir_limit_offset;
    float *boxes;
    float *scores;
    int32_t *labels;
} sad_anchor_decode_args;
int sad_anchor_decode_f32(const sad_anchor_decode_args *args, sad_stream_t stream);

typedef struct sad_center_decode_args {
    size_t struct_size;
    const float *hm, *reg, *height, *dim, *rot, *vel;
    const int32_t *index;
    int B, H, W, C, layout, P, log_dim, peak;
    float lo_x, lo_y, sx, sy;
    float *boxes, *scores;
    int32_t *labels;
} sad_center_decode_args;
int sad_center_decode_f32(const sad_center_decode_args *args, sad_stream_t stream);


typedef struct sad_anchor_targets_args {
    size_t struct_size;
    const float *gt_boxes;
    const int32_t *gt_labels;
    int B, G, D, H, W, ns, nr, nb;
    int use_size_class;
    float sizes[48];
    float z_center[16];
    float rotations[8];
    float pos_thr[16], neg_thr[16];
    int32_t size_class[16];
    float x0, y0, sx, sy;
    float dir_offset;
    int32_t *labels, *match;
    float *reg_target, *max_iou;
    int32_t *dir_target;
    void *workspace;
} sad_anchor_targets_args;
size_t sad_anchor_targets_workspace_bytes(int B, int G);
int sad_anchor_targets_f32(const sad_anchor_targets_args *args, sad_stream_t stream);

typedef struct sad_center_targets_args {
    size_t struct_size;
    const float *gt_boxes;
    const int32_t *gt_labels;
    int B, G, D, C, H, W, layout, min_radius, vel;
    float lo_x, lo_y, sx, sy, min_overlap;
    float *heatmap;
    int32_t *ind;
    float *anno;
} sad_center_targets_args;
int sad_center_targets_f32(const sad_center_targets_args *args, sad_stream_t stream);


typedef struct sad_anchor_head_loss_args {
    size_t struct_size;
    const float *cls, *reg, *dir;
    const int32_t *labels;
    const float *reg_target;
    const int32_t *dir_target;
    int B, H, W, A, C, nb, layout, sin_diff, normalize;
    float alpha, beta;
    float code_weights[7];
    float scale[3];
    float *loss;
    int32_t *num_pos;
    float *grad_cls, *grad_reg, *grad_dir;
    float *per_anchor;
    void *workspace;
} sad_anchor_head_loss_args;
size_t sad_anchor_head_loss_workspace_bytes(int B, int H, int W, int A);
int sad_anchor_head_loss_f32(const sad_anchor_head_loss_args *args, sad_stream_t stream);

typedef struct sad_center_head_loss_args {
    size_t struct_size;
    const float *hm, *reg, *height, *dim, *rot, *vel;
    const float *heatmap;
    const int32_t *ind;
    const float *anno;
    int B, H, W, C, G, layout, normalize;
    float code_weights[10];
    float scale[2];
    float *loss;
    int32_t *num_pos;
    float *grad_hm, *grad_reg, *grad_height, *grad_dim, *grad_rot, *grad_vel;
    void *workspace;
} sad_center_head_loss_args;
size_t sad_center_head_loss_workspace_bytes(int B, int H, int W, int G);
int sad_center_head_loss_f32(const sad_center_head_loss_args *args, sad_stream_t stream);

#define SAD_ROI_CLS_ROI_IOU 0
#define SAD_ROI_CLS_CLS 1

typedef struct sad_roi_targets_args {
    size_t struct_size;
    const float *rois;
    const int32_t *roi_count, *roi_labels;
    const float *gt_boxes;
    const int32_t *gt_labels;
    int B, R, D, G, Dg, S, fg_max, cls_mode;
    unsigned seed;
    float fg_thr, bg_lo, hard_ratio, reg_fg_thr, cls_fg_thr, cls_bg_thr;
    int32_t *index, *match, *labels;
    float *iou, *cls_target;
    int32_t *reg_valid;
    float *rois_s, *gt_local, *reg_target;
    void *workspace;
} sad_roi_targets_args;
size_t sad_roi_targets_workspace_bytes(int B, int R);
int sad_roi_targets_f32(const sad_roi_targets_args *args, sad_stream_t stream);

int sad_roi_decode_f32(const float *rois, int D, const float *reg, int B, int S, float *boxes, sad_stream_t stream);

typedef struct sad_roi_head_loss_args {
    size_t struct_size;
    const float *rcnn_cls;
    const float *rcnn_reg;
    const float *cls_target;
    const int32_t *reg_valid;
    const float *reg_target;
    const float *rois;
    const float *gt_local;
    int B, S, D, normalize;
    float beta;
    float code_weights[7];
    float scale[3];
    float *loss;
    int32_t *num;
// ... 12 lines not shown
```

Baseline: 8498.

## Fuse candidate decode with multi-radius ball query and trim launch overhead

Adds a fused cluster_front kernel that decodes candidate centers and radii and runs the multi-radius ball query in one pass, with the points held in registers, replacing the separate candidates and ball-query launches for small M3. It also lets the candidate MLP read strided row blocks directly instead of first copying prefix rows. It also folds the rowscan block-sum pass into the write kernel when group counts are small, saving one launch. The costs are more register pressure, redundant per-block summation work in the single-pass scan, and new paths to maintain.

```diff
diff --git a/3dsad-main_amd/_lib.py b/3dsad-main_amd/_lib.py
--- a/3dsad-main_amd/_lib.py
+++ b/3dsad-main_amd/_lib.py
@@ -233,6 +233,8 @@
     "sad_mlp_scratch_bytes": (ctypes.c_size_t, [ctypes.c_int, ctypes.c_int, ctypes.c_int, ctypes.c_int,
                                                ctypes.POINTER(ctypes.c_int)]),
     "sad_mlp_chain_f32": (ctypes.c_int, [ctypes.POINTER(MlpArgs), vp]),
+    "sad_mlp_chain_blocks_f32": (ctypes.c_int, [ctypes.POINTER(MlpArgs), ctypes.c_int, ctypes.c_int, vp]),
+    "sad_mlp_rowscan_launches": (ctypes.c_int, [ctypes.c_longlong]),
     "sad_mlp_chain_multi_f32": (ctypes.c_int, [ctypes.POINTER(ctypes.POINTER(MlpArgs)), ctypes.c_int, vp]),
     "sad_mlp_packed_bytes_bf16": (ctypes.c_size_t, [ctypes.c_int, ctypes.POINTER(ctypes.c_int), ctypes.c_int]),
     "sad_mlp_pack_bf16": (ctypes.c_int, [ctypes.c_int, ctypes.POINTER(ctypes.c_int), ctypes.c_int,
@@ -243,6 +245,10 @@
     "sad_candidates_f32": (ctypes.c_int, [vp, vp, ctypes.c_int, ctypes.c_int, ctypes.c_int,
                                          ctypes.c_float, ctypes.c_float, ctypes.c_float, c_f32p,
                                          vp, vp, vp]),
+    "sad_cluster_front_f32": (ctypes.c_int, [vp, vp, ctypes.c_int, ctypes.c_int, ctypes.c_int,
+                                            ctypes.c_float, ctypes.c_float, ctypes.c_float, c_f32p,
+                                            ctypes.c_int, c_f32p, ctypes.POINTER(ctypes.c_int),
+                                            vp, vp, ctypes.POINTER(vp), ctypes.POINTER(vp), vp]),
     "sad_nms_bev_f32": (ctypes.c_int, [vp, ctypes.c_int, ctypes.c_int, ctypes.c_float, ctypes.c_float,
                                       vp, vp, vp, vp]),
     "sad_nms_bev_workspace_bytes": (ctypes.c_size_t, [ctypes.c_int, ctypes.c_int]),
@@ -283,7 +289,8 @@
 
 def is_launch(name: str) -> bool:
     return (name.startswith("sad_") and not name.endswith(("_bytes", "_floats", "_bytes_bf16"))
-            and "preferred_geometry" not in name and name not in ("sad_version", "sad_last_error", "sad_set_option", "sad_mlp_padded_dims"))
+            and "preferred_geometry" not in name and name not in ("sad_version", "sad_last_error", "sad_set_option", "sad_mlp_padded_dims",
+                                                                        "sad_mlp_rowscan_launches"))
 
 
 def build(force: bool = False) -> str:
diff --git a/3dsad-main_amd/csrc/api.hip b/3dsad-main_amd/csrc/api.hip
--- a/3dsad-main_amd/csrc/api.hip
+++ b/3dsad-main_amd/csrc/api.hip
@@ -36,6 +36,7 @@
     if (!strcmp(key, "mlp_steal_after")) { sad::g_opt[sad::OPT_MLP_STEAL_AFTER].store(value, std::memory_order_relaxed); return SAD_OK; }
     if (!strcmp(key, "mlp_layer_queue")) { sad::g_opt[sad::OPT_MLP_LAYER_QUEUE].store(value, std::memory_order_relaxed); return SAD_OK; }
     if (!strcmp(key, "mlp_rows_form")) { sad::g_opt[sad::OPT_MLP_ROWS_FORM].store(value, std::memory_order_relaxed); return SAD_OK; }
+    if (!strcmp(key, "mlp_scan_two")) { sad::g_opt[sad::OPT_MLP_SCAN_TWO].store(value, std::memory_order_relaxed); return SAD_OK; }
     if (!strcmp(key, "mlp_check_inuse")) { sad::g_opt[sad::OPT_MLP_CHECK_INUSE].store(value, std::memory_order_relaxed); return SAD_OK; }
     if (!strcmp(key, "group_variant")) { sad::g_opt[sad::OPT_GROUP_VARIANT].store(value, std::memory_order_relaxed); return SAD_OK; }
     if (!strcmp(key, "bq_variant")) { sad::g_opt[sad::OPT_BQ_VARIANT].store(value, std::memory_order_relaxed); return SAD_OK; }
diff --git a/3dsad-main_amd/csrc/cluster_front.hip b/3dsad-main_amd/csrc/cluster_front.hip
--- /dev/null
+++ b/3dsad-main_amd/csrc/cluster_front.hip
@@ -0,0 +1,151 @@
+#include "common.h"
+
+namespace {
+
+struct CFParams {
+    float scale[SAD_MAX_RADII];
+    int nsample[SAD_MAX_RADII];
+    int32_t *idx[SAD_MAX_RADII];
+    int32_t *cnt[SAD_MAX_RADII];
+    float anchor[3];
+    float shift_max, r_min, r_max;
+};
+
+constexpr int CF_WAVES = 4;
+constexpr int CF_CPW = 4;
+constexpr int CF_MAX_POINTS = 2048;
+
+template <int NR, int PPL>
+__global__ __launch_bounds__(CF_WAVES * 64) void cluster_front_kernel(const float *__restrict__ xyz3, const float *__restrict__ c,
+                                                                      CFParams prm, int M3, int K, float *__restrict__ cand,
+                                                                      float *__restrict__ radius) {
+    const int lane = threadIdx.x & 63;
+    const int wave = __builtin_amdgcn_readfirstlane(threadIdx.x >> 6);
+    const int b = blockIdx.y;
+    const int m0 = (blockIdx.x * CF_WAVES + wave) * CF_CPW;
+    if (m0 >= K) return;
+    const float *p = xyz3 + (size_t)b * M3 * 3;
+    const int nchunks = (M3 + 63) >> 6;
+
+    float px[PPL], py[PPL], pz[PPL];
+#pragma unroll
+    for (int i = 0; i < PPL; ++i) {
+        const int j = i * 64 + lane;
+        const int jj = j < M3 ? j : M3 - 1;
+        px[i] = p[jj * 3 + 0];
+        py[i] = p[jj * 3 + 1];
+        pz[i] = p[jj * 3 + 2];
+    }
+
+    const int m1 = m0 + CF_CPW < K ? m0 + CF_CPW : K;
+    for (int m = m0; m < m1; ++m) {
+        const float *ci = c + ((size_t)b * K + m) * 6;
+        const float *q = p + m * 3;
+        float ctr[3], sz[3];
+#pragma unroll
+        for (int d = 0; d < 3; ++d) {
+            float sh = ci[d];
+            sh = sh < -prm.shift_max ? -prm.shift_max : sh;
+            sh = sh > prm.shift_max ? prm.shift_max : sh;
+            ctr[d] = q[d] + sh;
+            float s = ci[3 + d];
+            s = s < -1.0f ? -1.0f : s;
+            s = s > 1.0f ? 1.0f : s;
+            const float t1 = s * s;
+            const float t2 = 0.5f * t1;
+            const float t3 = 1.0f + s;
+            const float qq = t3 + t2;
+            sz[d] = prm.anchor[d] * qq;
+        }
+        const float ll = sz[0] * sz[0], ww = sz[1] * sz[1], hh = sz[2] * sz[2];
+        float sum = ll + ww;
+        sum = sum + hh;
+        float r = 0.5f * sqrtf(sum);
+        r = r < prm.r_min ? prm.r_min : r;
+        r = r > prm.r_max ? prm.r_max : r;
+        const size_t g = (size_t)b * K + m;
+        if (lane < 3) cand[g * 3 + lane] = lane == 0 ? ctr[0] : (lane == 1 ? ctr[1] : ctr[2]);
+        if (lane == 3) radius[g] = r;
+
+        float r2[NR], r2max = -__builtin_inff();
+        int cnt[NR], first[NR], ndone = 0;
+#pragma unroll
+        for (int k = 0; k < NR; ++k) {
+            const float rad = prm.scale[k] * r;
+            r2[k] = rad * rad;
+            r2max = r2[k] > r2max ? r2[k] : r2max;
+            cnt[k] = 0;
+            first[k] = 0;
+        }
+#pragma unroll
+        for (int i = 0; i < PPL; ++i) {
+            if (i >= nchunks || ndone >= NR) break;
+            const int j = i * 64 + lane;
+            const bool valid = j < M3;
+            const float d = sad::d2f(px[i], py[i], pz[i], ctr[0], ctr[1], ctr[2]);
+            if (__ballot(valid && (d < r2max)) == 0ull) continue;
+#pragma unroll
+            for (int k = 0; k < NR; ++k) {
+                const bool in = valid && (d < r2[k]);
+                const unsigned long long mask = __ballot(in);
+                const int S = prm.nsample[k];
+                if (mask != 0ull && cnt[k] < S) {
+                    const int slot = cnt[k] + __builtin_amdgcn_mbcnt_hi((unsigned)(mask >> 32), __builtin_amdgcn_mbcnt_lo((unsigned)mask, 0u));
+                    if (in && slot < S) prm.idx[k][g * S + slot] = j;
+                    if (cnt[k] == 0) first[k] = i * 64 + __builtin_ctzll(mask);
+                    cnt[k] += __builtin_popcountll(mask);
+                    if (cnt[k] >= S) ++ndone;
+                }
+            }
+        }
+#pragma unroll
+        for (int k = 0; k < NR; ++k) {
+            const int S = prm.nsample[k];
+            const int n = cnt[k] < S ? cnt[k] : S;
+            for (int s = n + lane; s < S; s += 64) prm.idx[k][g * S + s] = first[k];
+            if (lane == 0) prm.cnt[k][g] = n;
+        }
+    }
+}
+
+template <int NR>
+void launch_cf(const float *xyz3, const float *c, const CFParams &prm, int B, int M3, int K, float *cand, float *radius, hipStream_t st) {
+    const dim3 grid((K + CF_WAVES * CF_CPW - 1) / (CF_WAVES * CF_CPW), B), block(CF_WAVES * 64);
+    if (M3 <= 512) hipLaunchKernelGGL((cluster_front_kernel<NR, 8>), grid, block, 0, st, xyz3, c, prm, M3, K, cand, radius);
+    else if (M3 <= 1024) hipLaunchKernelGGL((cluster_front_kernel<NR, 16>), grid, block, 0, st, xyz3, c, prm, M3, K, cand, radius);
+    else hipLaunchKernelGGL((cluster_front_kernel<NR, 32>), grid, block, 0, st, xyz3, c, prm, M3, K, cand, radius);
+}
+
+}
+
+SAD_API int sad_cluster_front_f32(const float *xyz3, const float *c, int B, int M3, int K, float shift_max, float r_min,
+                                  float r_max, const float *anchor, int n_radii, const float *scales, const int *nsamples,
+                                  float *cand, float *radius, int32_t *const *idx, int32_t *const *cnt, sad_stream_t stream) {
+    SAD_REQUIRE(xyz3 && c && anchor && cand && radius, "sad_cluster_front_f32: NULL pointer");
+    SAD_REQUIRE(B >= 1 && B <= 65535 && K >= 1 && K <= M3, "sad_cluster_front_f32: need 1 <= B <= 65535, 1 <= K <= M3 (B=%d K=%d M3=%d)", B, K, M3);
+    SAD_REQUIRE(n_radii >= 1 && n_radii <= SAD_MAX_RADII, "sad_cluster_front_f32: n_radii=%d not in 1..%d", n_radii, SAD_MAX_RADII);
+    SAD_REQUIRE(scales && nsamples && idx && cnt, "sad_cluster_front_f32: NULL parameter array");
+    CFParams prm{};
+    for (int r = 0; r < n_radii; ++r) {
+        SAD_REQUIRE(nsamples[r] >= 1 && nsamples[r] <= 64, "sad_cluster_front_f32: nsample=%d not in 1..64", nsamples[r]);
+        SAD_REQUIRE(idx[r] && cnt[r], "sad_cluster_front_f32: NULL idx / cnt output");
+        prm.scale[r] = scales[r];
+        prm.nsample[r] = nsamples[r];
+        prm.idx[r] = idx[r];
+        prm.cnt[r] = cnt[r];
+    }
+    if (M3 > CF_MAX_POINTS)
+        return sad::fail(SAD_EUNSUPPORTED, "sad_cluster_front_f32: M3=%d > %d (use sad_candidates_f32 + sad_ball_query_multi_f32)", M3, CF_MAX_POINTS);
+    for (int d = 0; d < 3; ++d) prm.anchor[d] = anchor[d];
+    prm.shift_max = shift_max;
+    prm.r_min = r_min;
+    prm.r_max = r_max;
+    hipStream_t st = (hipStream_t)stream;
+    switch (n_radii) {
+        case 1: launch_cf<1>(xyz3, c, prm, B, M3, K, cand, radius, st); break;
+        case 2: launch_cf<2>(xyz3, c, prm, B, M3, K, cand, radius, st); break;
+        case 3: launch_cf<3>(xyz3, c, prm, B, M3, K, cand, radius, st); break;
+        default: launch_cf<4>(xyz3, c, prm, B, M3, K, cand, radius, st); break;
+    }
+    return sad::check_launch("sad_cluster_front_f32");
+}
diff --git a/3dsad-main_amd/csrc/common.h b/3dsad-main_amd/csrc/common.h
--- a/3dsad-main_amd/csrc/common.h
+++ b/3dsad-main_amd/csrc/common.h
@@ -44,7 +44,7 @@
 constexpr int CONT_BIT = 1 << 29;
 constexpr int GID_MASK = CONT_BIT - 1;
 constexpr int SCAN_MAX_CHAINS = SAD_MAX_RADII;
-struct ScanMulti { ScanJob j[SCAN_MAX_CHAINS]; int n; };
+struct ScanMulti { ScanJob j[SCAN_MAX_CHAINS]; int n, single; };
 ScanJob make_scan_job(const int32_t *cnt, int ngroups, int S, int R, int *tab, int nodedup, const int32_t *idx, int N, int M);
 int launch_rowscan_multi(const ScanJob *jobs, int n, hipStream_t st);
 int launch_rowscan(const int32_t *cnt, int ngroups, int S, int R, int *tab, hipStream_t st, int nodedup = 0,
@@ -157,7 +157,7 @@
 long long bfreg_stream_frags(int shape);
 int bfreg_pack(int shape, const int *dims, int first_has_xyz, const float *const *W, void *dst, hipStream_t st);
 int launch_bfreg(const BfRegMulti &mp, hipStream_t st);
-enum { OPT_FPS_DPP = 0, OPT_MLP_RW = 1, OPT_MLP_BUDGET_KB = 2, OPT_BQ_VARIANT = 3, OPT_FPS_VARIANT = 4, OPT_MLP_FORCE = 5, OPT_MLP_DEDUP_F = 6, OPT_MLP_NODEDUP = 7, OPT_FPS_THREADS = 8, OPT_MLP_STATIC = 9, OPT_GROUP_VARIANT = 10, OPT_MLP_DYN_SLOTS = 11, OPT_MLP_NOXCD = 12, OPT_MLP_STEAL_AFTER = 13, OPT_MLP_CHECK_INUSE = 14, OPT_MLP_LAYER_QUEUE = 15, OPT_MLP_ROWS_FORM = 16, OPT_NN_VARIANT = 17, OPT_SPCONV_GRAD_RANGES = 18, OPT_COUNT };
+enum { OPT_FPS_DPP = 0, OPT_MLP_RW = 1, OPT_MLP_BUDGET_KB = 2, OPT_BQ_VARIANT = 3, OPT_FPS_VARIANT = 4, OPT_MLP_FORCE = 5, OPT_MLP_DEDUP_F = 6, OPT_MLP_NODEDUP = 7, OPT_FPS_THREADS = 8, OPT_MLP_STATIC = 9, OPT_GROUP_VARIANT = 10, OPT_MLP_DYN_SLOTS = 11, OPT_MLP_NOXCD = 12, OPT_MLP_STEAL_AFTER = 13, OPT_MLP_CHECK_INUSE = 14, OPT_MLP_LAYER_QUEUE = 15, OPT_MLP_ROWS_FORM = 16, OPT_NN_VARIANT = 17, OPT_SPCONV_GRAD_RANGES = 18, OPT_MLP_SCAN_TWO = 19, OPT_COUNT };
 
 inline int fail(int code, const char *fmt, ...) {
     char buf[480];
diff --git a/3dsad-main_amd/csrc/mlp_chain.h b/3dsad-main_amd/csrc/mlp_chain.h
--- a/3dsad-main_amd/csrc/mlp_chain.h
+++ b/3dsad-main_amd/csrc/mlp_chain.h
@@ -40,6 +40,7 @@
     int *rowtab;
     const int *row_src, *row_gid;
     long long total_groups;
+    int blk_rows, blk_stride;
 };
 
 constexpr int MULTI_MAX = 4;
diff --git a/3dsad-main_amd/csrc/mlp_chain.hip b/3dsad-main_amd/csrc/mlp_chain.hip
--- a/3dsad-main_amd/csrc/mlp_chain.hip
+++ b/3dsad-main_amd/csrc/mlp_chain.hip
@@ -286,7 +286,7 @@
             } else {
                 long long gr = r0 + r;
                 if (gr >= p.total_rows) gr = p.total_rows - 1;
-                sm_idx[r] = (int)gr;
+                sm_idx[r] = p.blk_rows ? (int)(gr / p.blk_rows * p.blk_stride + gr % p.blk_rows) : (int)gr;
             }
         }
         __syncthreads();
diff --git a/3dsad-main_amd/csrc/mlp_dispatch.hip b/3dsad-main_amd/csrc/mlp_dispatch.hip
--- a/3dsad-main_amd/csrc/mlp_dispatch.hip
+++ b/3dsad-main_amd/csrc/mlp_dispatch.hip
@@ -404,6 +404,20 @@
     return launch_prepared(q, (hipStream_t)stream);
 }
 
+SAD_API int sad_mlp_chain_blocks_f32(const sad_mlp_args *a, int rows_per_block, int block_stride, sad_stream_t stream) {
+    SAD_REQUIRE(!a || !a->idx, "sad_mlp_chain_blocks_f32: plain rows only (idx must be NULL)");
+    Prepared q;
+    if (int e = prepare_chain(a, stream, q)) return e;
+    if (q.kind != TILED)
+        return sad::fail(SAD_EUNSUPPORTED, "sad_mlp_chain_blocks_f32: the tiled kernel only (geometry 0 or a W / WN / RW code)");
+    SAD_REQUIRE(rows_per_block >= 1 && block_stride >= rows_per_block && q.p.total_rows % rows_per_block == 0,
+                "sad_mlp_chain_blocks_f32: need 1 <= rows_per_block=%d <= block_stride=%d and B*M=%lld a multiple of rows_per_block",
+                rows_per_block, block_stride, q.p.total_rows);
+    SAD_REQUIRE(q.p.total_rows / rows_per_block * block_stride < (1LL << 31), "sad_mlp_chain_blocks_f32: too many source rows");
+    if (rows_per_block != block_stride) { q.p.blk_rows = rows_per_block; q.p.blk_stride = block_stride; }
+    return launch_prepared(q, (hipStream_t)stream);
+}
+
 SAD_API int sad_mlp_chain_multi_f32(const sad_mlp_args *const *args, int n, sad_stream_t stream) {
     SAD_REQUIRE(args && n >= 1, "sad_mlp_chain_multi_f32: need at least one chain");
     hipStream_t st = (hipStream_t)stream;
diff --git a/3dsad-main_amd/csrc/mlp_rowscan.hip b/3dsad-main_amd/csrc/mlp_rowscan.hip
--- a/3dsad-main_amd/csrc/mlp_rowscan.hip
+++ b/3dsad-main_amd/csrc/mlp_rowscan.hip
@@ -7,6 +7,7 @@
 constexpr int SCAN_T = 256;
 constexpr int SCAN_LOG = 8;
 constexpr int SCAN_WAVES = SCAN_T / 64;
+constexpr int SCAN_SINGLE_MAX = 32768;
 static_assert(SCAN_T == 1 << SCAN_LOG, "the row search of rowscan_write_kernel is SCAN_LOG halvings");
 
 __device__ __forceinline__ int scan_job_of(const sad::ScanMulti &sm, int block, int &local) {
@@ -47,7 +48,12 @@
     const sad::ScanJob &jb = sm.j[scan_job_of(sm, blockIdx.x, lb)];
     const int tid = threadIdx.x, lane = tid & 63, wave = tid >> 6;
     int part = 0;
-    for (int b = tid; b < lb; b += SCAN_T) part += jb.blk_sum[b];
+    if (sm.single) {
+#pragma unroll 4
+        for (int gp = tid; gp < lb * SCAN_T; gp += SCAN_T) part += clamp_cnt(jb, gp);
+    } else {
+        for (int b = tid; b < lb; b += SCAN_T) part += jb.blk_sum[b];
+    }
     for (int off = 32; off >= 1; off >>= 1) part += __shfl_xor(part, off, 64);
     if (lane == 0) wsum[wave] = part;
     __syncthreads();
@@ -74,6 +80,7 @@
     if (tid == SCAN_T - 1) s_start[SCAN_T] = run + c;
     __syncthreads();
     const int blk_rows = s_start[SCAN_T];
+    if (sm.single && tid == 0) jb.blk_sum[lb] = blk_rows;
     if (jb.split) {
         if (g < jb.ngroups) jb.gstart[g] = base + run;
         if (g == jb.ngroups - 1) jb.gstart[jb.ngroups] = base + run + c;
@@ -169,13 +176,15 @@
 int launch_rowscan_multi(const ScanJob *jobs, int n, hipStream_t st) {
     ScanMulti sm{};
     sm.n = n;
+    sm.single = get_option(OPT_MLP_SCAN_TWO) ? 0 : 1;
     int blocks = 0;
     for (int i = 0; i < n; ++i) {
         sm.j[i] = jobs[i];
         sm.j[i].blk0 = blocks;
         blocks += (jobs[i].ngroups + SCAN_T - 1) / SCAN_T;
-    }
-    hipLaunchKernelGGL(rowscan_sums_kernel, dim3(blocks), dim3(SCAN_T), 0, st, sm);
+        if (jobs[i].ngroups > SCAN_SINGLE_MAX) sm.single = 0;
+    }
+    if (!sm.single) hipLaunchKernelGGL(rowscan_sums_kernel, dim3(blocks), dim3(SCAN_T), 0, st, sm);
     hipLaunchKernelGGL(rowscan_write_kernel, dim3(blocks), dim3(SCAN_T), 0, st, sm);
 #ifdef SAD_SCAN_TWICE
     hipLaunchKernelGGL(rowscan_sums_kernel, dim3(blocks), dim3(SCAN_T), 0, st, sm);
@@ -241,6 +250,10 @@
     return rowscan_entry("sad_mlp_rowscan_split", SCAN_SPLIT, a, stream);
 }
 
+SAD_API int sad_mlp_rowscan_launches(long long ngroups) {
+    return (ngroups <= SCAN_SINGLE_MAX && !sad::get_option(sad::OPT_MLP_SCAN_TWO)) ? 1 : 2;
+}
+
 SAD_API size_t sad_mlp_cont_bytes(int B, int M, int S, int cout) {
     if (B < 1 || M < 1 || S < 1 || cout < 1) return 0;
     const size_t tiles = ((size_t)B * M * S + 31) / 32;
diff --git a/3dsad-main_amd/detector.py b/3dsad-main_amd/detector.py
--- a/3dsad-main_amd/detector.py
+++ b/3dsad-main_amd/detector.py
@@ -359,14 +359,13 @@
             cur_xyz = new_xyz
         K = cfg.n_cand
         M3 = cur_xyz.shape[1]
-        c = self.cand_mlp.rows(cur_feat if K == M3 else ops.prefix_rows(cur_feat, K))
-        cand = ops._empty((B, K, 3), dtype=torch.float32, device=points.device)
-        rad = ops._empty((B, K), dtype=torch.float32, device=points.device)
-        check(lib().sad_candidates_f32(cur_xyz.data_ptr(), c.data_ptr(), B, M3, K, cfg.shift_max,
-                                       cfg.r_min, cfg.r_max, self._anchor, cand.data_ptr(),
-                                       rad.data_ptr(), main.cuda_stream), "sad_candidates_f32")
-        idxs, cnts = ops.ball_query_multi(cfg.cluster_scales, cfg.cluster_nsamples, cur_xyz, cand, rad,
-                                          return_counts=True)
+        fused = ops.FUSED_CLUSTER_FRONT
+        if K != M3 and fused and isinstance(self.cand_mlp, ops.PackedMLP):
+            c = self.cand_mlp.rows(cur_feat, blocks=(K, M3))
+        else:
+            c = self.cand_mlp.rows(cur_feat if K == M3 else ops.prefix_rows(cur_feat, K))
+        cand, rad, idxs, cnts = ops.cluster_front(cur_xyz, c, cfg.cluster_scales, cfg.cluster_nsamples, cfg.shift_max, cfg.r_min,
+                                                  cfg.r_max, self._anchor, fused=None if fused else False)
         cat = cats[-1]
         ckont = conts[-1]
         if cat is None and trace is None and not ops.AUTOTUNE and self._cluster_can_split(B):
@@ -381,6 +380,12 @@
             outs, o_ = [], 0
             for mlp, k_ in zip(self.cluster_branches, ckont):
                 outs.append((cat, o_, mlp.out_channels, k_))
+                o_ += mlp.out_channels
+            cwss = ops.rowscan_multi(idxs, cnts, M3, outs)
+        elif fused and not ops.AUTOTUNE and cat.dtype == torch.float32 and self._cluster_tables(B):
+            outs, o_ = [], 0
+            for mlp in self.cluster_branches:
+                outs.append((cat, o_, mlp.out_channels))
                 o_ += mlp.out_channels
             cwss = ops.rowscan_multi(idxs, cnts, M3, outs)
         for mlp, idx, cnt, ws, k_ in zip(self.cluster_branches, idxs, cnts, cwss, ckont or [None] * len(idxs)):
diff --git a/3dsad-main_amd/mlp.py b/3dsad-main_amd/mlp.py
--- a/3dsad-main_amd/mlp.py
+++ b/3dsad-main_amd/mlp.py
@@ -388,13 +388,30 @@
         a.scratch, a.scratch_bytes = sc.data_ptr(), nbytes
         keep.append(sc)
 
-    def rows(self, x: torch.Tensor, out: Optional[torch.Tensor] = None, col_off: int = 0
-             ) -> torch.Tensor:
+    def rows(self, x: torch.Tensor, out: Optional[torch.Tensor] = None, col_off: int = 0,
+             blocks: Optional[Tuple[int, int]] = None) -> torch.Tensor:
         if self.first_has_xyz:
             raise RuntimeError("this PackedMLP was packed with the xyz prefix")
         if not x.is_cuda or x.dtype != torch.float32:
             raise TypeError("x: expected a GPU float32 tensor")
         ops._on_current_device(x, "x")
+        if blocks is not None and tuple(blocks)[0] != tuple(blocks)[1]:
+            K, M = (int(v) for v in blocks)
+            if x.dim() != 3 or x.shape[1] != M or not 1 <= K <= M or not x.is_contiguous():
+                raise ValueError(f"rows: blocks=({K}, {M}) needs a contiguous [B,{M},C] tensor and 1 <= K <= M")
+            if out is not None or col_off:
+                raise ValueError("rows: blocks comes without out / col_off")
+            x2, _, C = self._rows_input(x)
+            a = self._args()
+            out = ops._empty((x.shape[0], K, self.out_channels), dtype=torch.float32, device=x.device)
+            self._rows_args(a, x2, out, 0)
+            a.M = x.shape[0] * K
+            a.geometry = self._geom.get(self._key(a)) or self.default_geometry
+            if ops.AUTOTUNE or 1 <= a.geometry % 1000 <= 5:
+                return self.rows(ops.prefix_rows(x, K))
+            _dispatch(self.name, "sad_mlp_chain_blocks_f32",
+                      lambda: lib().sad_mlp_chain_blocks_f32(ctypes.byref(a), K, M, ops._stream()), [x2, out])
+            return out
         x2, R, C = self._rows_input(x)
         if out is None:
             out = ops._empty(tuple(x.shape[:-1]) + (self.out_channels,), dtype=torch.float32,
diff --git a/3dsad-main_amd/ops.py b/3dsad-main_amd/ops.py
--- a/3dsad-main_amd/ops.py
+++ b/3dsad-main_amd/ops.py
@@ -70,6 +70,7 @@
 AUTOTUNE: bool = False
 MERGE_BF16: bool = True
 SPLIT_POOL: bool = not os.environ.get("SAD_NO_SPLIT_POOL")
+FUSED_CLUSTER_FRONT: bool = not os.environ.get("SAD_NO_CLUSTER_FRONT")
 
 
 class _timed:
@@ -310,6 +311,44 @@
         check(lib().sad_ball_query_multi_f32(xyz.data_ptr(), new_xyz.data_ptr(), n, r_arr, pc, s_arr,
                                              p_arr, c_arr, B, N, M, _stream()), "sad_ball_query_multi_f32")
     return (outs, cnts) if return_counts else outs
+
+
+CLUSTER_FRONT_MAX_POINTS = 2048
+CLUSTER_FRONT_AUTO_POINTS = 512
+
+
+def cluster_front(xyz3: torch.Tensor, c: torch.Tensor, scales: Sequence[float], nsamples: Sequence[int], shift_max: float,
+                  r_min: float, r_max: float, anchor: Sequence[float], fused: Optional[bool] = None):
+    xyz3 = _need(xyz3, "xyz3", torch.float32, 3)
+    c = _need(c, "c", torch.float32, 3)
+    B, M3, _ = xyz3.shape
+    K = c.shape[1]
+    n = len(scales)
+    if c.shape[0] != B or c.shape[2] != 6 or xyz3.shape[2] != 3 or not 1 <= K <= M3:
+        raise ValueError(f"cluster_front: expected xyz3 [B,M3,3] and c [B,K,6] with 1 <= K <= M3, got {tuple(xyz3.shape)}, {tuple(c.shape)}")
+    if n != len(nsamples) or not 1 <= n <= _lib.MAX_RADII:
+        raise ValueError(f"need 1..{_lib.MAX_RADII} scales with matching nsamples")
+    a_arr = anchor if isinstance(anchor, ctypes.Array) else (ctypes.c_float * 3)(*[_f32(v) for v in anchor])
+    cand = _empty((B, K, 3), dtype=torch.float32, device=xyz3.device)
+    rad = _empty((B, K), dtype=torch.float32, device=xyz3.device)
+    if fused is None:
+        fused = FUSED_CLUSTER_FRONT and M3 <= CLUSTER_FRONT_AUTO_POINTS
+    if not fused or M3 > CLUSTER_FRONT_MAX_POINTS:
+        check(lib().sad_candidates_f32(xyz3.data_ptr(), c.data_ptr(), B, M3, K, _f32(shift_max), _f32(r_min), _f32(r_max), a_arr,
+                                       cand.data_ptr(), rad.data_ptr(), _stream()), "sad_candidates_f32")
+        idxs, cnts = ball_query_multi(scales, nsamples, xyz3, cand, rad, return_counts=True)
+        return cand, rad, idxs, cnts
+    idxs = [_empty((B, K, int(s)), dtype=torch.int32, device=xyz3.device) for s in nsamples]
+    cnts = [_empty((B, K), dtype=torch.int32, device=xyz3.device) for _ in nsamples]
+    r_arr = (ctypes.c_float * n)(*[_f32(r) for r in scales])
+    s_arr = (ctypes.c_int * n)(*[int(s) for s in nsamples])
+    p_arr = (vp * n)(*[o.data_ptr() for o in idxs])
+    c_arr = (vp * n)(*[o.data_ptr() for o in cnts])
+    with _timed("ball_query", f"N{M3}M{K}x{n}"):
+        check(lib().sad_cluster_front_f32(xyz3.data_ptr(), c.data_ptr(), B, M3, K, _f32(shift_max), _f32(r_min), _f32(r_max), a_arr,
+                                          n, r_arr, s_arr, cand.data_ptr(), rad.data_ptr(), p_arr, c_arr, _stream()),
+              "sad_cluster_front_f32")
+    return cand, rad, idxs, cnts
 
 
 def knn_query(k: int, xyz: torch.Tensor, new_xyz: torch.Tensor) -> torch.Tensor:
diff --git a/include/sad_amd.h b/include/sad_amd.h
--- a/include/sad_amd.h
+++ b/include/sad_amd.h
@@ -189,10 +189,12 @@
 int sad_mlp_rowscan_init(int n, const int32_t *const *cnt, const int32_t *const *idx, const int *S, int B, int N,
                          int M, void *const *workspace, float *const *out, const int *ld_out, const int *col_off,
                          const int *cout, sad_stream_t stream);
+int sad_mlp_rowscan_launches(long long ngroups);
 size_t sad_mlp_scratch_bytes(int B, int M, int S, int L, const int *dims);
 int sad_mlp_preferred_geometry(int L, const int *dims);
 int sad_mlp_padded_dims(int L, const int *dims, int *padded);
 int sad_mlp_chain_f32(const sad_mlp_args *args, sad_stream_t stream);
+int sad_mlp_chain_blocks_f32(const sad_mlp_args *args, int rows_per_block, int block_stride, sad_stream_t stream);
 int sad_mlp_chain_multi_f32(const sad_mlp_args *const *args, int n, sad_stream_t stream);
 
 size_t sad_mlp_packed_bytes_bf16(int L, const int *dims, int first_has_xyz);
@@ -236,6 +238,9 @@
 int sad_candidates_f32(const float *xyz3, const float *c, int B, int M3, int K, float shift_max,
                        float r_min, float r_max, const float *anchor, float *cand, float *radius,
                        sad_stream_t stream);
+int sad_cluster_front_f32(const float *xyz3, const float *c, int B, int M3, int K, float shift_max, float r_min, float r_max,
+                          const float *anchor, int n_radii, const float *scales, const int *nsamples, float *cand,
+                          float *radius, int32_t *const *idx, int32_t *const *cnt, sad_stream_t stream);
 int sad_decode_boxes_f32(const float *cand, const float *o, int B, int K, const float *anchors,
                          float *boxes, sad_stream_t stream);
 
```

Result: no change. 8507, median of 2 (+0.1%).
